# tomzzy1/ldbc_graphalytics_platforms_graphblas

Hardware: AMD Instinct MI355X
Metric: edges/sec (GTEPS) per algorithm at 1/2/4/8 GPUs; % HBM roofline (higher is better)
Workload: dtype f64; 1 GPU; PageRank SYN-8_5 (R-MAT scale 23, ef 40, seed 85, undirected); algorithm=pagerank, graph=SYN-8_5, n=8388608, nnz=628313590, parallelism=row1, partition=one rank, driver=device, hipGraph, exchange=device copies, roofline_events=timed steps, device=AMD Radeon Graphics (gfx950:sramecc+:xnack-), cus=256

## Files before the change

### ldbc_graphalytics_platforms_graphblas_amd/csrc/gx_pr.h

```cpp
#pragma once

#include <chrono>
#include <cstdio>
#include <cstdlib>
#include <vector>

#include <algorithm>

#include "gx_device.h"

namespace gx {

struct PlanClock {
    bool on = false, sync = true;
    hipStream_t s = nullptr;
    const char *what = "";
    std::chrono::steady_clock::time_point t;
    PlanClock(const char *w, hipStream_t st) : s(st), what(w) {
        const char *e = std::getenv("GX_PLAN_TIMES");
        on = e && std::atoi(e) != 0;
        sync = !(e && std::atoi(e) == 2);
        if (on) {
            if (sync) (void)hipStreamSynchronize(s);
            t = std::chrono::steady_clock::now();
        }
    }
    void mark(const char *phase) {
        if (!on) return;
        if (sync) (void)hipStreamSynchronize(s);
        const auto now = std::chrono::steady_clock::now();
        std::fprintf(stderr, "[plan %s] %-28s %8.2f ms\n", what, phase,
                     std::chrono::duration<double, std::milli>(now - t).count());
        t = now;
    }
};

struct RowBlock {
    int64_t nz_begin;
    int64_t nz_end;
    int32_t row_begin;
    int32_t row_end;
    int32_t split;
    int32_t seg;
};

struct SortedUnit {
    int64_t lo;
    int64_t hi;
    int64_t step;
    int64_t slab;
    int64_t nbeg;
    int32_t nsg;
    int32_t blk;
    int32_t part;
    int32_t unit;
    int32_t nunits;
    int32_t seg;
    int64_t z0, z1;
    int32_t r0, r1;
    int64_t pbeg;
    int32_t psg;
    int32_t pad;
};

struct CombStripe {
    int64_t slab;
    int32_t r0, nrows, s0, s1, k, dslot;
};

__device__ __forceinline__ void store_x(double *x_out, double *xd, int64_t live, int64_t row, double v) {
    if (row < live) x_out[row] = v;
    else xd[row - live] = v;
}

constexpr int kPullBlock = 256;
constexpr int kStreamNnz = 2048;
constexpr int kStreamRows = 256;
constexpr int kSegNnz = 8192;

struct PrPart {
    gx_ctx *ctx = nullptr;
    uint64_t n_global = 0;
    int nranks = 1, rank = 0;
    uint64_t rows = 0;
    uint64_t chunk = 0;
    uint64_t live = ~0ull;
    DBuf<double> xd;
    double damping = 0.85;
    DBuf<int64_t> rp_own;
    DBuf<int32_t> ci_own;
    const int64_t *rp = nullptr;
    const int32_t *ci = nullptr;
    DBuf<int32_t> outdeg_own;
    const int32_t *outdeg = nullptr;
    DBuf<RowBlock> blocks;
    uint32_t nblocks = 0;
    uint32_t nlong_blocks = 0;
    DBuf<int32_t> long_first;
    DBuf<int32_t> long_nseg;
    DBuf<double> long_part;
    DBuf<uint32_t> long_ticket;
    uint32_t nlong = 0, nsegs = 0;
    DBuf<int32_t> dlist;
    uint64_t nd = 0;
    bool d_range = false;
    int64_t d0 = 0;
    uint32_t dgrid = 0;
    DBuf<double> dpart;
    DBuf<uint32_t> dticket;
    DBuf<int32_t> sci;
    DBuf<uint32_t> spk;
    DBuf<uint32_t> gbase;
    DBuf<uint16_t> npk;
    DBuf<uint32_t> nbase;
    uint64_t nnarrow = 0;
    uint64_t ncodes = 0;
    uint32_t null_sg = 0;
    DBuf<uint32_t> ppk;
    DBuf<uint32_t> pbase;
    uint64_t npair = 0;
    uint64_t npfill = 0;
    uint64_t npslots = 0;
    uint32_t pnull_sg = 0;
    int sorted_nnz = 65536;
    int sorted_rows = 4096;
    int64_t unit_nnz = 0;
    DBuf<SortedUnit> units;
    uint32_t nunits = 0;
    DBuf<double> uslab;
    DBuf<uint32_t> uticket;
    bool comb_kernel = false;
    bool force_huge = false;
    DBuf<CombStripe> cstripes;
    uint32_t ncstripes = 0;
    DBuf<uint64_t> utimes;
    int utimes_launch = 0;
    int long_nnz = 65536;
    int sorted_lds = 0;
    int cache_policy = 0;
    uint32_t nt_col = 65536;
    uint32_t nsorted = 0, nlong_pad = 0;
    bool rows_desc = false;
    int queue_on = -1;
    DBuf<uint32_t> queue;
    bool fused_dangling = false;
    DBuf<int32_t> dslot;
    DBuf<double> fdpart;
    DBuf<uint32_t> fdticket;
    uint32_t ndblocks = 0;
    uint32_t iso_units = 0, iso_dblocks = 0;
    uint64_t iso_rows = 0;
    int kernel = 2;
    const int64_t *src_rp = nullptr;
    const int32_t *src_ci = nullptr;
    const int32_t *src_order = nullptr;
    const int32_t *src_perm = nullptr;
    UploadJob *job = nullptr;
    DBuf<int32_t> order;
    DBuf<double> xa, xb, rank_out, result;
    DBuf<int32_t> perm;
};

struct LengthRuns {
    std::vector<int64_t> pos, val, base;
    uint64_t n = 0;
    int64_t total = 0;
    size_t run(uint64_t i) const {
        return (size_t)(std::upper_bound(pos.begin(), pos.end(), (int64_t)i) - pos.begin()) - 1;
    }
    int64_t prefix(uint64_t i) const {
        if (i >= n) return total;
        const size_t k = run(i);
        return base[k] + ((int64_t)i - pos[k]) * val[k];
    }
    int64_t length(uint64_t i) const { return val[run(i)]; }
};

template <typename T>
struct HostView {
    const T *p = nullptr;
    size_t n = 0;
    const LengthRuns *runs = nullptr;
    bool prefix = false;
    template <typename Alloc>
    HostView(const std::vector<T, Alloc> &v) : p(v.data()), n(v.size()) {}
    HostView(const T *ptr, size_t count) : p(ptr), n(count) {}
    HostView(const LengthRuns *r, bool pre) : n(pre ? r->n + 1 : r->n), runs(r), prefix(pre) {}
    size_t size() const { return n; }
    T operator[](size_t i) const { return p ? p[i] : (T)(prefix ? runs->prefix(i) : runs->length(i)); }
};

int pr_plan(PrPart *p, HostView<int64_t> h_rp, const int64_t *d_rp,
            const int32_t *d_ci, const int32_t *d_outdeg, HostView<int32_t> h_outdeg);

int pr_plan_sorted(PrPart *p, HostView<int64_t> h_rp, HostView<int32_t> h_outdeg);
int pr_step_sorted(PrPart *p, const double *x_full, double *x_local, double *rank_out, hipStream_t s);
int pr_dangling(PrPart *p, double *x_local, hipStream_t s);

int pr_init(PrPart *p, double *x_local, hipStream_t s);
int pr_single_plan(gx_graph *g, PrPart **out);
constexpr int kPlanBlockRows = 16320;
constexpr int64_t kPlanBlockNnz = 32 << 20;

struct MultiBlocks {
    std::vector<std::vector<int32_t>> pos;
    std::vector<int32_t> slot;
    uint64_t chunk = 0;
    std::vector<int32_t> order, perm;
};
int pr_multi_blocks(const gx_csr *A, int directed, int ndev, MultiBlocks *out);
int pr_multi_interleave(const gx_csr *A, int ndev, MultiBlocks *out);

int pr_multi_plan(gx_graph *g, int ndev, int d, uint64_t chunk, double damping, const MultiBlocks *mb,
                  PrPart **out);
int pr_part_build(gx_ctx *ctx, uint64_t n_global, int nranks, int rank, uint64_t chunk, uint64_t live,
                  const std::vector<int64_t> &h_rp, const std::vector<int32_t> &ci, const std::vector<int32_t> &h_outdeg,
                  double damping, PrPart **out, bool force_huge = false);
int pr_part_build_rows(gx_ctx *ctx, const gx_csr *A, int nranks, int rank, uint64_t chunk,
                       const std::vector<int32_t> &rows, const int32_t *colmap, double damping, bool force_huge,
                       PrPart **out);
int pr_step(PrPart *p, const double *x_full, double *x_local, double *rank_out, hipStream_t s);

}
```

### ldbc_graphalytics_platforms_graphblas_amd/csrc/gx_pr_sorted.hip

```cpp
#include <algorithm>
#include <functional>
#include <queue>
#include <thread>
#include <type_traits>
#include <cstdio>
#include <cstdlib>
#include <cstring>

#include "gx_pr.h"
#include "gx_pr_bank.h"

namespace gx {
namespace {

constexpr int kRowBits = 14;
constexpr int kBS = 1024;
constexpr int kCombRows = (1 << kRowBits) / kBS;
constexpr int kU = 8;
constexpr int kRound = kBS * kU;
constexpr int kNSg = 512;
constexpr int kPSg = 256;
constexpr int kJunkRow = (1 << kRowBits) - kWave;
constexpr int kMaxBlockRows = kJunkRow;
static_assert(kMaxBlockRows == kPlanBlockRows, "gx_pr.h block rows");

struct SortedArgs {
    const RowBlock *blocks;
    const int32_t *ci;
    const int32_t *sci;
    const uint32_t *spk;
    const uint32_t *gbase;
    const int32_t *outdeg;
    const double *x_in;
    double *x_out;
    double *rank_out;
    int64_t chunk;
    int nranks;
    int zero_slot;
    int32_t zero_col;
    double teleport0, damping_over_n, damping;
    const int32_t *long_first;
    const int32_t *long_nseg;
    double *long_part;
    uint32_t *long_ticket;
    uint32_t nlong, nlong_pad;
    const int32_t *dslot;
    double *dpart;
    uint32_t *dticket;
    uint32_t ndblocks;
    double iso_rows;
    const SortedUnit *units;
    uint32_t nunits;
    double *uslab;
    uint32_t *uticket;
    uint64_t *utimes;
    const uint16_t *npk;
    const uint32_t *nbase;
    uint32_t null_sg;
    uint32_t nt_col;
    const uint32_t *ppk;
    const uint32_t *pbase;
    uint32_t pnull_sg;
    double *xd;
    int64_t live;
    uint32_t *queue;
    int comb;
    const CombStripe *cstripes;
};

__device__ __forceinline__ double sorted_epilogue(const SortedArgs &a, int64_t row, double s, double teleport) {
    const double r = teleport + s;
    if (a.rank_out) a.rank_out[row] = r;
    const int32_t deg = a.outdeg[row];
    store_x(a.x_out, a.xd, a.live, row, deg > 0 ? r / ((double)deg / a.damping) : r);
    return deg > 0 ? 0.0 : r;
}

__device__ __forceinline__ double epilogue_rows(const SortedArgs &a, int64_t r0, int nrows, const double *acc,
                                                double teleport) {
    constexpr int kB = 8;
    double d = 0.0;
    for (int i0 = threadIdx.x; i0 < nrows; i0 += kB * kBS) {
        int32_t deg[kB];
#pragma unroll
        for (int q = 0; q < kB; q++) {
            const int i = i0 + q * kBS;
            deg[q] = i < nrows ? a.outdeg[r0 + i] : 1;
        }
#pragma unroll
        for (int q = 0; q < kB; q++) {
            const int i = i0 + q * kBS;
            if (i >= nrows) break;
            const double r = teleport + (acc ? acc[i] : 0.0);
            if (a.rank_out) a.rank_out[r0 + i] = r;
            store_x(a.x_out, a.xd, a.live, r0 + i, deg[q] > 0 ? r / ((double)deg[q] / a.damping) : r);
            if (deg[q] == 0) d += r;
        }
    }
    return d;
}

template <int BS = kBS>
__device__ __forceinline__ void dangling_publish(const SortedArgs &a, int32_t slot, double d, double *wred, int *last,
                                                 double teleport) {
    const int tid = threadIdx.x;
    d = wave_sum(d);
    __syncthreads();
    if ((tid & (kWave - 1)) == 0) wred[tid / kWave] = d;
    __syncthreads();
    if (tid == 0) {
        double tot = 0.0;
#pragma unroll
        for (int w = 0; w < BS / kWave; w++) tot += wred[w];
        __hip_atomic_store(&a.dpart[slot], tot, __ATOMIC_RELAXED, __HIP_MEMORY_SCOPE_AGENT);
        __builtin_amdgcn_fence(__ATOMIC_RELEASE, "agent");
        asm volatile("s_waitcnt vmcnt(0)" ::: "memory");
        const uint32_t t = __hip_atomic_fetch_add(a.dticket, 1u, __ATOMIC_RELAXED, __HIP_MEMORY_SCOPE_AGENT);
        *last = t == a.ndblocks - 1;
    }
    __syncthreads();
    if (!*last) return;
    __builtin_amdgcn_fence(__ATOMIC_ACQUIRE, "agent");
    double v = 0.0;
    for (uint32_t j = tid; j < a.ndblocks; j += BS) v += __hip_atomic_load(&a.dpart[j], __ATOMIC_RELAXED, __HIP_MEMORY_SCOPE_AGENT);
    v = wave_sum(v);
    __syncthreads();
    if ((tid & (kWave - 1)) == 0) wred[tid / kWave] = v;
    __syncthreads();
    if (tid == 0) {
        double all = 0.0;
#pragma unroll
        for (int w = 0; w < BS / kWave; w++) all += wred[w];
        __hip_atomic_store(a.dticket, 0u, __ATOMIC_RELAXED, __HIP_MEMORY_SCOPE_AGENT);
        a.x_out[a.chunk - 1] = all + a.iso_rows * teleport;
    }
}

__device__ __forceinline__ void long_segment(const SortedArgs &a, const RowBlock &b, double *wred, double teleport) {
    const int tid = threadIdx.x;
    const int64_t zb = b.nz_begin, ze = b.nz_end;
    double s0 = 0.0, s1 = 0.0;
    for (int64_t k0 = zb + tid; k0 < ze; k0 += (int64_t)kU * kBS) {
        int32_t c[kU];
#pragma unroll
        for (int u = 0; u < kU; u++) c[u] = __builtin_nontemporal_load(a.ci + min(k0 + (int64_t)u * kBS, ze - 1));
        double g[kU];
#pragma unroll
        for (int u = 0; u < kU; u++) g[u] = a.x_in[c[u]];
#pragma unroll
        for (int u = 0; u < kU; u++)
            if (k0 + (int64_t)u * kBS < ze) ((u & 1) ? s1 : s0) += g[u];
    }
    const double s = wave_sum(s0 + s1);
    if ((tid & (kWave - 1)) == 0) wred[tid / kWave] = s;
    __syncthreads();
    if (tid != 0) return;
    double tot = 0.0;
#pragma unroll
    for (int w = 0; w < kBS / kWave; w++) tot += wred[w];
    const int32_t sp = b.split;
    const int32_t nseg = a.long_nseg[sp];
    if (nseg == 1) {
        sorted_epilogue(a, b.row_begin, tot, teleport);
        return;
    }
    const int32_t first = a.long_first[sp];
    __hip_atomic_store(&a.long_part[first + b.seg], tot, __ATOMIC_RELAXED, __HIP_MEMORY_SCOPE_AGENT);
    __builtin_amdgcn_fence(__ATOMIC_RELEASE, "agent");
    asm volatile("s_waitcnt vmcnt(0)" ::: "memory");
    const uint32_t t = __hip_atomic_fetch_add(&a.long_ticket[sp], 1u, __ATOMIC_RELAXED, __HIP_MEMORY_SCOPE_AGENT);
    if (t != (uint32_t)(nseg - 1)) return;
    __builtin_amdgcn_fence(__ATOMIC_ACQUIRE, "agent");
    double all = 0.0;
    for (int j = 0; j < nseg; j++)
        all += __hip_atomic_load(&a.long_part[first + j], __ATOMIC_RELAXED, __HIP_MEMORY_SCOPE_AGENT);
    __hip_atomic_store(&a.long_ticket[sp], 0u, __ATOMIC_RELAXED, __HIP_MEMORY_SCOPE_AGENT);
    sorted_epilogue(a, b.row_begin, all, teleport);
}

template <int CP>
__device__ __forceinline__ void gather_units(const SortedArgs &a, const RowBlock &b, int64_t lo64, int64_t hi64,
                                             double *acc, int64_t step64) {
    const int tid = threadIdx.x;
    const int64_t z0 = b.nz_begin;
    const int32_t lo = (int32_t)(lo64 - z0), hi = (int32_t)(hi64 - z0), step = (int32_t)step64;
    if (lo >= hi) return;
    const int32_t last = (int32_t)(b.nz_end - z0) - 1;
    const int32_t nsg = (last >> 8) + 1;
    const uint32_t span = (uint32_t)(hi - lo);
    const uint32_t *spk = a.spk + z0;
    const int32_t *sci = a.sci + z0;
    const uint32_t *sgb = a.gbase + b.seg;
    const int32_t zc = a.zero_col;
    const char *xb = reinterpret_cast<const char *>(a.x_in);
    const int lane = tid & (kWave - 1);
    constexpr int V = kU / 4;
    const int wave = tid >> 6;
    struct Rd {
        uint4 q[V];
        uint32_t bq;
    };
    struct Gt {
        double g[kU];
        uint32_t r[kU];
    };
    auto load = [&](Rd &d, int32_t R) {
        const int32_t sg0 = R + wave * V * 256;
#pragma unroll
        for (int v = 0; v < V; v++) {
            const int32_t sg = sg0 + v * 256;
            const gx_u32x4 *qa = reinterpret_cast<const gx_u32x4 *>(spk + min(sg + 4 * lane, last));
            const gx_u32x4 q4 = (CP & 1) ? __builtin_nontemporal_load(qa) : *qa;
            d.q[v] = make_uint4(q4.x, q4.y, q4.z, q4.w);
        }
        d.bq = sgb[min((sg0 >> 8) + (lane & (V - 1)), nsg - 1)];
    };
    auto issue = [&](const Rd &d, int32_t R, Gt &t) {
        int32_t c[kU];
        uint32_t sb[V], esc = 0;
#pragma unroll
        for (int v = 0; v < V; v++) {
            sb[v] = __builtin_amdgcn_readlane(d.bq, v);
            esc |= sb[v];
        }
#pragma unroll
        for (int v = 0; v < V; v++) {
            const uint32_t w4[4] = {d.q[v].x, d.q[v].y, d.q[v].z, d.q[v].w};
            const int32_t d0 = R + (wave * V + v) * 256 + 4 * lane - lo;
            const uint32_t base = sb[v] & 0x7fffffffu;
#pragma unroll
            for (int j = 0; j < 4; j++) {
                const int i = 4 * v + j;
                const bool ok = (uint32_t)(d0 + j) < span;
                t.r[i] = w4[j] & ((1u << kRowBits) - 1);
                asm volatile("" : "+v"(t.r[i]));
                c[i] = ok ? (int32_t)(base + (w4[j] >> kRowBits)) : zc;
            }
        }
        if (esc & 0x80000000u) {
#pragma unroll
            for (int v = 0; v < V; v++) {
                if (!(sb[v] & 0x80000000u)) continue;
#pragma unroll
                for (int j = 0; j < 4; j++) {
                    const int i = 4 * v + j;
                    const int32_t pos = R + (wave * V + v) * 256 + 4 * lane + j;
                    if ((uint32_t)(pos - lo) < span) c[i] = sci[pos];
                }
            }
            __builtin_amdgcn_s_waitcnt(0x0f70);
        }
#pragma unroll
        for (int i = 0; i < kU; i++) t.g[i] = *reinterpret_cast<const double *>(xb + ((uint32_t)c[i] << 3));
    };
    auto add = [&](const Gt &t) {
#pragma unroll
        for (int i = 0; i < kU; i++) atomicAdd(&acc[t.r[i]], t.g[i]);
    };
    const int32_t nr = (hi - lo + step - 1) / step;
    if (nr <= 0) return;
    Rd dA, dB;
    Gt tA, tB;
    int32_t R = lo;
    load(dA, R);
    load(dB, R + step);
    issue(dA, R, tA);
    __builtin_amdgcn_sched_barrier(0);
    load(dA, R + 2 * step);
    int32_t k = 1;
    for (; k + 1 < nr; k += 2) {
        __builtin_amdgcn_sched_barrier(0);
        issue(dB, R + step, tB);
        __builtin_amdgcn_sched_barrier(0);
        load(dB, R + 3 * step);
        __builtin_amdgcn_sched_barrier(0);
        add(tA);
        __builtin_amdgcn_sched_barrier(0);
        issue(dA, R + 2 * step, tA);
        __builtin_amdgcn_sched_barrier(0);
        load(dA, R + 4 * step);
        __builtin_amdgcn_sched_barrier(0);
        add(tB);
        R += 2 * step;
    }
    if (k < nr) {
        issue(dB, R + step, tB);
        add(tA);
        add(tB);
    } else {
        add(tA);
    }
}

__device__ __forceinline__ uint32_t wave_scan_incl(uint32_t v) {
    v += (uint32_t)__builtin_amdgcn_update_dpp(0, (int)v, 0x111, 0xf, 0xf, false);
    v += (uint32_t)__builtin_amdgcn_update_dpp(0, (int)v, 0x112, 0xf, 0xf, false);
    v += (uint32_t)__builtin_amdgcn_update_dpp(0, (int)v, 0x114, 0xf, 0xf, false);
    v += (uint32_t)__builtin_amdgcn_update_dpp(0, (int)v, 0x118, 0xf, 0xf, false);
    v += (uint32_t)__builtin_amdgcn_update_dpp(0, (int)v, 0x142, 0xa, 0xf, false);
    v += (uint32_t)__builtin_amdgcn_update_dpp(0, (int)v, 0x143, 0xc, 0xf, false);
    return v;
}

template <int CP>
__device__ __forceinline__ void gather_narrow(const SortedArgs &a, const SortedUnit &u, double *acc) {
    constexpr int W = kBS / kWave;
    const int32_t nrounds = (u.nsg + W - 1) / W;
    if (u.unit >= nrounds) return;
    const int32_t nr = (nrounds - u.unit + u.nunits - 1) / u.nunits;
    if (nr <= 0) return;
    const int tid = threadIdx.x;
    const int lane = tid & (kWave - 1);
    const int wave = tid >> 6;
    const uint32_t sg0 = (uint32_t)(u.nbeg / kNSg);
    const char *xb = reinterpret_cast<const char *>(a.x_in);
    typedef uint32_t u32x4 __attribute__((ext_vector_type(4)));
    struct Rd {
        u32x4 q;
        uint32_t base;
    };
    struct Gt {
        double g[kU];
        uint32_t r[kU];
    };
    auto load = [&](Rd &d, int32_t i) {
        const int32_t sg = (u.unit + i * u.nunits) * W + wave;
        const uint32_t g = sg < u.nsg ? sg0 + (uint32_t)sg : a.null_sg;
        const u32x4 *qa = reinterpret_cast<const u32x4 *>(a.npk + (size_t)g * kNSg) + lane;
        d.q = (CP & 1) ? __builtin_nontemporal_load(qa) : *qa;
        d.base = a.nbase[g];
    };
    auto issue = [&](const Rd &d, Gt &t) {
        const uint32_t w[4] = {d.q.x, d.q.y, d.q.z, d.q.w};
        uint32_t pk[2] = {0u, 0u};
#pragma unroll
        for (int k = 0; k < kU; k++) {
            const uint32_t c = (k & 1) ? (w[k >> 1] >> 16) : (w[k >> 1] & 0xffffu);
            pk[k >> 2] |= (c >> kRowBits) << (8 * (k & 3));
            t.r[k] = c & ((1u << kRowBits) - 1);
            asm volatile("" : "+v"(t.r[k]));
        }
        const uint32_t s0 = wave_scan_incl(pk[0]), s1 = wave_scan_incl(pk[1]);
        const uint32_t t0 = (uint32_t)__builtin_amdgcn_readlane((int)s0, kWave - 1);
        const uint32_t t1 = (uint32_t)__builtin_amdgcn_readlane((int)s1, kWave - 1);
        uint32_t bk = (uint32_t)__builtin_amdgcn_readfirstlane((int)d.base);
        const uint32_t b0 = bk;
        uint32_t col[kU];
#pragma unroll
        for (int k = 0; k < kU; k++) {
            const uint32_t sk = k < 4 ? s0 : s1, tk = k < 4 ? t0 : t1;
            col[k] = bk + ((sk >> (8 * (k & 3))) & 255u);
            bk += (tk >> (8 * (k & 3))) & 255u;
        }
        if ((CP & 4) && b0 >= a.nt_col) {
#pragma unroll
            for (int k = 0; k < kU; k++) t.g[k] = __builtin_nontemporal_load(reinterpret_cast<const double *>(xb + (col[k] << 3)));
        } else {
#pragma unroll
            for (int k = 0; k < kU; k++) t.g[k] = *reinterpret_cast<const double *>(xb + (col[k] << 3));
        }
    };
    auto add = [&](const Gt &t) {
#pragma unroll
        for (int k = 0; k < kU; k++) atomicAdd(&acc[t.r[k]], t.g[k]);
    };
    Rd dA, dB;
    Gt tA, tB;
    load(dA, 0);
    load(dB, 1);
    issue(dA, tA);
    __builtin_amdgcn_sched_barrier(0);
    load(dA, 2);
    int32_t k = 1;
    for (; k + 1 < nr; k += 2) {
        __builtin_amdgcn_sched_barrier(0);
        issue(dB, tB);
        __builtin_amdgcn_sched_barrier(0);
        load(dB, k + 2);
        __builtin_amdgcn_sched_barrier(0);
        add(tA);
        __builtin_amdgcn_sched_barrier(0);
        issue(dA, tA);
        __builtin_amdgcn_sched_barrier(0);
        load(dA, k + 3);
        __builtin_amdgcn_sched_barrier(0);
        add(tB);
    }
    if (k < nr) {
        issue(dB, tB);
        add(tA);
        add(tB);
    } else {
        add(tA);
    }
}

template <int CP>
__device__ __forceinline__ void gather_pairs(const SortedArgs &a, const SortedUnit &u, double *acc) {
    constexpr int W = kBS / kWave;
    constexpr int kS = kU / 2;
    const int32_t nrounds = (u.psg + W - 1) / W;
    if (u.unit >= nrounds) return;
    const int32_t nr = (nrounds - u.unit + u.nunits - 1) / u.nunits;
    const int tid = threadIdx.x;
    const int lane = tid & (kWave - 1);
    const int wave = tid >> 6;
    const uint32_t sg0 = (uint32_t)(u.pbeg / kPSg);
    const char *xb = reinterpret_cast<const char *>(a.x_in);
    typedef uint32_t u32x4 __attribute__((ext_vector_type(4)));
    typedef double d2 __attribute__((ext_vector_type(2)));
    struct Rd {
        u32x4 q;
        uint32_t base;
    };
    struct Gt {
        d2 g[kS];
        uint32_t r[kS];
    };
    auto load = [&](Rd &d, int32_t i) {
        const int32_t sg = (u.unit + i * u.nunits) * W + wave;
        const uint32_t g = sg < u.psg ? sg0 + (uint32_t)sg : a.pnull_sg;
        const u32x4 *qa = reinterpret_cast<const u32x4 *>(a.ppk + (size_t)g * kPSg) + lane;
        d.q = (CP & 1) ? __builtin_nontemporal_load(qa) : *qa;
        d.base = a.pbase[g];
    };
    auto issue = [&](const Rd &d, Gt &t) {
        const uint32_t w[kS] = {d.q.x, d.q.y, d.q.z, d.q.w};
        uint32_t pk = 0u;
#pragma unroll
        for (int k = 0; k < kS; k++) {
            pk |= (w[k] >> 30) << (8 * k);
            t.r[k] = w[k] & 0x3fffffffu;
            asm volatile("" : "+v"(t.r[k]));
        }
        const uint32_t sc = wave_scan_incl(pk);
        const uint32_t tot = (uint32_t)__builtin_amdgcn_readlane((int)sc, kWave - 1);
        uint32_t bk = (uint32_t)__builtin_amdgcn_readfirstlane((int)d.base);
        const uint32_t b0 = bk;
        uint32_t pr[kS];
#pragma unroll
        for (int k = 0; k < kS; k++) {
            pr[k] = bk + ((sc >> (8 * k)) & 255u);
            bk += (tot >> (8 * k)) & 255u;
        }
        if ((CP & 4) && 2u * b0 >= a.nt_col) {
#pragma unroll
            for (int k = 0; k < kS; k++) t.g[k] = __builtin_nontemporal_load(reinterpret_cast<const d2 *>(xb + (pr[k] << 4)));
        } else {
#pragma unroll
            for (int k = 0; k < kS; k++) t.g[k] = *reinterpret_cast<const d2 *>(xb + (pr[k] << 4));
        }
    };
    auto add = [&](const Gt &t) {
#pragma unroll
        for (int k = 0; k < kS; k++) {
            const uint32_t r = t.r[k];
            atomicAdd(&acc[(r >> 15) & ((1u << kRowBits) - 1)], (r & (1u << 29)) ? t.g[k].y : t.g[k].x);
            atomicAdd(&acc[r & ((1u << kRowBits) - 1)], (r & (1u << kRowBits)) ? t.g[k].y : t.g[k].x);
        }
    };
    Rd dA, dB;
    Gt tA, tB;
    load(dA, 0);
    load(dB, 1);
    issue(dA, tA);
    __builtin_amdgcn_sched_barrier(0);
    load(dA, 2);
    int32_t k = 1;
    for (; k + 1 < nr; k += 2) {
        __builtin_amdgcn_sched_barrier(0);
        issue(dB, tB);
        __builtin_amdgcn_sched_barrier(0);
        load(dB, k + 2);
        __builtin_amdgcn_sched_barrier(0);
        add(tA);
        __builtin_amdgcn_sched_barrier(0);
        issue(dA, tA);
        __builtin_amdgcn_sched_barrier(0);
        load(dA, k + 3);
        __builtin_amdgcn_sched_barrier(0);
        add(tB);
    }
    if (k < nr) {
        issue(dB, tB);
        add(tA);
        add(tB);
    } else {
        add(tA);
    }
}

template <bool TIMES, int CP>
__device__ __forceinline__ void pull_item(const SortedArgs &a, const uint32_t w, double *acc, double *wred, int &last,
                                          const double teleport) {
    const int tid = threadIdx.x;
    __shared__ uint64_t ts[2];
    if (TIMES && tid == 0) ts[0] = __builtin_amdgcn_s_memrealtime();
    auto stamp = [&]() {
        if (TIMES && tid == 0) {
            a.utimes[4 * w + 0] = ts[0];
            a.utimes[4 * w + 1] = ts[1];
            a.utimes[4 * w + 2] = __builtin_amdgcn_s_memrealtime();
            a.utimes[4 * w + 3] = (uint64_t)__builtin_amdgcn_s_getreg((3 << 11) | 20);
        }
    };
    if (a.zero_slot && w == 0 && tid == 0) a.x_out[a.chunk - 1] = a.iso_rows * teleport;
    if (w < a.nlong_pad) {
        if (w < a.nlong) long_segment(a, a.blocks[w], wred, teleport);
        stamp();
        return;
    }
    const SortedUnit u = a.units[w - a.nlong_pad];
    const RowBlock b = {u.z0, u.z1, u.r0, u.r1, -1, u.seg};
    const int nrows = b.row_end - b.row_begin;
    const bool empty = b.nz_begin == b.nz_end;
    if (!empty) {
        for (int i = tid; i < nrows; i += kBS) acc[i] = 0.0;
        __syncthreads();
        gather_pairs<CP>(a, u, acc);
        gather_narrow<CP>(a, u, acc);
        gather_units<CP>(a, b, u.lo, u.hi, acc, u.step);
        __syncthreads();
    }
    if (TIMES && tid == 0) ts[1] = __builtin_amdgcn_s_memrealtime();
    if (u.nunits > 1 && a.comb) {
        double *mine = a.uslab + u.slab + (int64_t)u.unit * nrows;
        for (int i = tid; i < nrows; i += kBS) mine[i] = acc[i];
        stamp();
        return;
    }
    if (u.nunits > 1) {
        double *mine = a.uslab + u.slab + (int64_t)u.unit * nrows;
        for (int i = tid; i < nrows; i += kBS)
            __hip_atomic_store(&mine[i], acc[i], __ATOMIC_RELAXED, __HIP_MEMORY_SCOPE_AGENT);
        asm volatile("s_waitcnt vmcnt(0)" ::: "memory");
        __syncthreads();
        if (tid == 0) {
            const uint32_t t = __hip_atomic_fetch_add(&a.uticket[u.part], 1u, __ATOMIC_RELAXED, __HIP_MEMORY_SCOPE_AGENT);
            last = t == (uint32_t)(u.nunits - 1);
            if (last) {
                __builtin_amdgcn_fence(__ATOMIC_ACQUIRE, "agent");
                asm volatile("s_waitcnt vmcnt(0)" ::: "memory");
                __hip_atomic_store(&a.uticket[u.part], 0u, __ATOMIC_RELAXED, __HIP_MEMORY_SCOPE_AGENT);
            }
        }
        __syncthreads();
        if (!last) {
            stamp();
            return;
        }
        const double *slabs = a.uslab + u.slab;
        if (2 * nrows <= kBS) {
            int S = 2;
            while (4 * S * nrows <= 2 * kBS && S < u.nunits) S *= 2;
            double *part = acc + (1 << (kRowBits - 1));
            const int r = tid % nrows, g = tid / nrows;
            if (g < S) {
                double s = 0.0;
                for (int j0 = g; j0 < u.nunits; j0 += kCombRows * S) {
                    double v[kCombRows];
#pragma unroll
                    for (int q = 0; q < kCombRows; q++) {
                        const int j = j0 + q * S;
                        v[q] = j < u.nunits ? slabs[(int64_t)j * nrows + r] : 0.0;
                    }
#pragma unroll
                    for (int q = 0; q < kCombRows; q++) s += v[q];
                }
                part[g * nrows + r] = s;
            }
            __syncthreads();
            if (tid < nrows) {
                double s = 0.0;
                for (int q = 0; q < S; q++) s += part[q * nrows + tid];
                acc[tid] = s;
            }
        } else
        for (int i0 = tid; i0 < nrows; i0 += kCombRows * kBS) {
            double s[kCombRows];
#pragma unroll
            for (int q = 0; q < kCombRows; q++) s[q] = 0.0;
            for (int j = 0; j < u.nunits; j++) {
                const double *sl = slabs + (int64_t)j * nrows;
                double v[kCombRows];
#pragma unroll
                for (int q = 0; q < kCombRows; q++) v[q] = i0 + q * kBS < nrows ? sl[i0 + q * kBS] : 0.0;
#pragma unroll
                for (int q = 0; q < kCombRows; q++) s[q] += v[q];
            }
#pragma unroll
            for (int q = 0; q < kCombRows; q++)
                if (i0 + q * kBS < nrows) acc[i0 + q * kBS] = s[q];
        }
    }
    double d = 0.0;
    if (empty)
        d = epilogue_rows(a, b.row_begin, nrows, nullptr, teleport);
    else
        d = epilogue_rows(a, b.row_begin, nrows, acc, teleport);
    if (a.dslot) {
        const int32_t slot = a.dslot[u.blk];
        if (slot >= 0) dangling_publish(a, slot, d, wred, &last, teleport);
    }
    stamp();
}

constexpr int kCombBS = 256;
__global__ __launch_bounds__(kCombBS) void k_pr_combine(SortedArgs a) {
    __shared__ double part[kCombBS];
    __shared__ double wred[kCombBS / kWave];
    __shared__ int last;
    double dsum = 0.0;
    for (int k = 0; k < a.nranks; k++) dsum += a.x_in[(int64_t)k * a.chunk + a.chunk - 1];
    const double teleport = a.teleport0 + a.damping_over_n * dsum;
    const CombStripe c = a.cstripes[blockIdx.x];
    const int rows = c.s1 - c.s0;
    int S = 1;
    while (2 * S * rows <= kCombBS && S < c.k) S *= 2;
    const int tid = threadIdx.x, r = tid % rows, g = tid / rows;
    double s = 0.0;
    if (g < S) {
        const double *sl = a.uslab + c.slab + c.s0 + r;
        for (int j0 = g; j0 < c.k; j0 += 16 * S) {
            double v[16];
#pragma unroll
            for (int q = 0; q < 16; q++) {
                const int j = j0 + q * S;
                v[q] = j < c.k ? sl[(int64_t)j * c.nrows] : 0.0;
            }
#pragma unroll
            for (int q = 0; q < 16; q++) s += v[q];
        }
    }
    if (S > 1) {
        if (g < S) part[g * rows + r] = s;
        __syncthreads();
        if (tid < rows) {
            s = 0.0;
            for (int q = 0; q < S; q++) s += part[q * rows + tid];
        }
    }
    double d = 0.0;
    if (tid < rows) d = sorted_epilogue(a, (int64_t)c.r0 + c.s0 + tid, s, teleport);
    if (c.dslot >= 0) dangling_publish<kCombBS>(a, c.dslot, d, wred, &last, teleport);
}

__device__ __forceinline__ uint32_t queue_fetch(uint32_t *q, uint32_t *slot) {
    if (__builtin_amdgcn_readfirstlane(threadIdx.x) < (uint32_t)kWave) {
        const uint32_t v = __hip_atomic_fetch_add(q, (threadIdx.x & (kWave - 1)) == 0 ? 1u : 0u, __ATOMIC_RELAXED,
                                                  __HIP_MEMORY_SCOPE_AGENT);
        *slot = __builtin_amdgcn_readfirstlane(v);
    }
    __syncthreads();
    const uint32_t w = __builtin_amdgcn_readfirstlane(*slot);
    __syncthreads();
    return w;
}

template <bool TIMES, int CP = 0, bool QUEUE = false>
__global__ __launch_bounds__(kBS, TIMES ? 1 : 4) void k_pr_pull_units(SortedArgs a) {
    extern __shared__ double acc[];
    __shared__ double wred[kBS / kWave];
    __shared__ int last;
    double dsum = 0.0;
    for (int k = 0; k < a.nranks; k++) dsum += a.x_in[(int64_t)k * a.chunk + a.chunk - 1];
    const double teleport = a.teleport0 + a.damping_over_n * dsum;
    if constexpr (!QUEUE) {
        pull_item<TIMES, CP>(a, blockIdx.x, acc, wred, last, teleport);
    } else {
        __shared__ uint32_t item;
        const uint32_t total = a.nlong_pad + a.nunits;
        for (;;) {
            const uint32_t w = queue_fetch(a.queue, &item);
            if (w >= total) break;
            pull_item<TIMES, CP>(a, w, acc, wred, last, teleport);
        }
        if (threadIdx.x == 0 &&
            __hip_atomic_fetch_add(&a.queue[1], 1u, __ATOMIC_RELAXED, __HIP_MEMORY_SCOPE_AGENT) == gridDim.x - 1) {
            __hip_atomic_store(&a.queue[0], 0u, __ATOMIC_RELAXED, __HIP_MEMORY_SCOPE_AGENT);
            __hip_atomic_store(&a.queue[1], 0u, __ATOMIC_RELAXED, __HIP_MEMORY_SCOPE_AGENT);
        }
    }
}

using PullKernel = void (*)(SortedArgs);
template <bool QUEUE>
PullKernel pull_kernel(bool times, int cache_policy) {
    if (times) return k_pr_pull_units<true, 0, QUEUE>;
    if (cache_policy == 5) return k_pr_pull_units<false, 5, QUEUE>;
    if (cache_policy == 1) return k_pr_pull_units<false, 1, QUEUE>;
    return k_pr_pull_units<false, 0, QUEUE>;
}

struct KeySrc {
    const int64_t *rp;
    int64_t rows;
    const int64_t *srp;
    const int32_t *sci;
    const int32_t *order;
    const int32_t *perm;
    const int32_t *seg_row;
    int32_t nseg;
    int colbits;
    int32_t segmask;
};

__global__ __launch_bounds__(256) void k_row_seg(const int32_t *__restrict__ seg_row, int32_t nseg, int32_t *rowseg) {
    for (int32_t sg = blockIdx.x; sg < nseg; sg += gridDim.x)
        for (int32_t r = seg_row[sg] + threadIdx.x; r < seg_row[sg + 1]; r += 256) rowseg[r] = sg;
}

constexpr int kKeyU = 4;

template <typename K>
__global__ __launch_bounds__(256) void k_sorted_keys(KeySrc k, int64_t nnz, const int64_t *__restrict__ srow,
                                                     int64_t nslabs, const int32_t *__restrict__ rowseg,
                                                     K *__restrict__ keys, uint16_t *__restrict__ vals) {
    const int lane = threadIdx.x & (kWave - 1);
    const int64_t nw = (int64_t)gridDim.x * (256 / kWave);
    const int64_t nch = (nslabs + kKeyU - 1) / kKeyU;
    for (int64_t ch = ((int64_t)blockIdx.x * 256 + threadIdx.x) / kWave; ch < nch; ch += nw) {
        int32_t i[kKeyU], sg[kKeyU], c0[kKeyU];
        int64_t rpi[kKeyU], sp[kKeyU];
        const int64_t e0 = ch * kKeyU * kWave + lane;
#pragma unroll
        for (int u = 0; u < kKeyU; u++) {
            const int64_t sl = min(ch * kKeyU + u, nslabs - 1);
            i[u] = (int32_t)slab_row_of(k.rp, srow, k.rows, sl, min(e0 + u * kWave, nnz - 1), lane);
        }
#pragma unroll
        for (int u = 0; u < kKeyU; u++) {
            sg[u] = rowseg[i[u]];
            rpi[u] = k.rp[i[u]];
            sp[u] = k.srp[k.order ? k.order[i[u]] : i[u]];
        }
#pragma unroll
        for (int u = 0; u < kKeyU; u++) c0[u] = k.sci[sp[u] + (min(e0 + u * kWave, nnz - 1) - rpi[u])];
#pragma unroll
        for (int u = 0; u < kKeyU; u++) {
            const uint32_t c = (uint32_t)(k.perm ? k.perm[c0[u]] : c0[u]);
            const int64_t e = e0 + u * kWave;
            if (e < nnz) {
                keys[e] = ((K)(sg[u] & k.segmask) << k.colbits) | (K)c;
                vals[e] = (uint16_t)(i[u] - k.seg_row[sg[u]]);
            }
        }
    }
}

template <typename K>
__global__ __launch_bounds__(256) void k_scatter_keys(KeySrc k, int64_t n_src, const int64_t *__restrict__ ssrow,
                                                      int64_t sl0, int64_t sl1, int64_t nnz,
                                                      const int32_t *__restrict__ rowseg, K *__restrict__ keys,
                                                      uint16_t *__restrict__ vals) {
    const int lane = threadIdx.x & (kWave - 1);
    const int64_t nw = (int64_t)gridDim.x * (256 / kWave);
    const int64_t nslabs_src = (nnz + kWave - 1) / kWave;
    for (int64_t sl = sl0 + ((int64_t)blockIdx.x * 256 + threadIdx.x) / kWave; sl < sl1; sl += nw) {
        const int64_t e = sl * kWave + lane;
        const int64_t ee = min(e, nnz - 1);
        const int64_t u = slab_row_of(k.srp, ssrow, n_src, min(sl, nslabs_src - 1), ee, lane);
        const int32_t i = k.perm[u];
        const int32_t sg = rowseg[i];
        const int64_t dst = k.rp[i] + (ee - k.srp[u]);
        const uint32_t c = (uint32_t)k.perm[k.sci[ee]];
        if (e < nnz) {
            keys[dst] = ((K)(sg & k.segmask) << k.colbits) | (K)c;
            vals[dst] = (uint16_t)(i - k.seg_row[sg]);
        }
    }
}

struct SegDesc {
    int64_t z0, z1;
    int32_t gseg;
    int32_t pad;
};

constexpr int64_t kPackChunk = 4096;
struct PackChunk {
    int64_t z0;
    int32_t seg;
    int32_t pad;
};

template <typename K>
__global__ __launch_bounds__(256) void k_sorted_pack(const SegDesc *__restrict__ segs, const PackChunk *__restrict__ chunks,
                                                     int64_t nchunks, const K *__restrict__ keys,
                                                     const uint16_t *__restrict__ vals, uint32_t colmask,
                                                     int32_t *__restrict__ sci, uint32_t *__restrict__ spk,
                                                     uint32_t *__restrict__ gbase) {
    for (int64_t c = blockIdx.x; c < nchunks; c += gridDim.x) {
        const PackChunk pc = chunks[c];
        const SegDesc sg = segs[pc.seg];
        const int64_t z1 = min(pc.z0 + kPackChunk, sg.z1);
#pragma unroll 4
        for (int64_t g0 = pc.z0; g0 < z1; g0 += 256) {
            const int64_t e = g0 + threadIdx.x;
            const bool in = e < z1;
            const uint32_t col = in ? (uint32_t)keys[e] & colmask : 0u;
            if (in) sci[e] = (int32_t)col;
            if (sg.gseg < 0 || !in) continue;
            const int64_t q = (g0 - sg.z0) >> 8;
            const uint32_t base = (uint32_t)keys[g0] & colmask;
            const uint32_t lastc = (uint32_t)keys[min(g0 + 255, sg.z1 - 1)] & colmask;
            const bool esc = lastc - base >= (1u << (32 - kRowBits));
            const uint32_t row = vals[e];
            spk[e] = esc ? row : ((col - base) << kRowBits) | row;
            if (threadIdx.x == 0) gbase[sg.gseg + q] = esc ? (base | 0x80000000u) : base;
        }
    }
}

__global__ __launch_bounds__(256) void k_sorted_laneperm(const RowBlock *__restrict__ blocks, const uint32_t *__restrict__ nsplit,
                                                         uint32_t *spk, int32_t *sci) {
    const RowBlock b = blocks[blockIdx.y];
    const int64_t z0 = b.nz_begin + 256 * (int64_t)nsplit[blockIdx.y], ngroups = (b.nz_end - z0) >> 6;
    const int lane = threadIdx.x & (kWave - 1);
    const int64_t wave = ((int64_t)blockIdx.x * blockDim.x + threadIdx.x) / kWave;
    const int64_t waves = (int64_t)gridDim.x * blockDim.x / kWave;
    for (int64_t g = wave; g < ngroups; g += waves) {
        const int64_t e = z0 + (g << 6) + lane;
        const uint32_t p = spk[e];
        const int32_t c = sci[e];
        const uint32_t row = p & ((1u << kRowBits) - 1);
        const uint32_t key = ((row & 15u) << 1) | ((row >> 4) & 1u);
        uint32_t rank = 0;
        for (uint32_t k = 0; k < 32; k++) {
            const uint64_t m = __ballot(key == k);
            if (k < key) rank += (uint32_t)__popcll(m);
            else if (k == key) rank += (uint32_t)__popcll(m & ((1ull << lane) - 1ull));
        }
        const int64_t dst = z0 + (g << 6) + 4 * (rank >> 2) + (rank & 3);
        spk[dst] = p;
        sci[dst] = c;
    }
}

constexpr int kBankTile = 2048, kBankBS = 256, kBankPer = kBankTile / kBankBS;
__global__ __launch_bounds__(kBankBS) void k_bank_order(const RowBlock *__restrict__ blocks, const uint32_t *__restrict__ qsplit,
                                                        const uint32_t *__restrict__ nsplit, uint32_t *spk, int32_t *sci) {
    __shared__ uint32_t cnt2[kBankTile / 2][kBankClasses / 2];
    __shared__ int32_t wred[2][kBankBS / kWave];
    const RowBlock b = blocks[blockIdx.y];
    const int64_t z0 = b.nz_begin, N = b.nz_end - z0;
    const int64_t Nq = min(N, (int64_t)qsplit[blockIdx.y] << 8), Np = min(N, (int64_t)nsplit[blockIdx.y] << 8);
    const int64_t ntiles = (Np + kBankTile - 1) / kBankTile;
    const int tid = threadIdx.x, lane = tid & (kWave - 1), wave = tid / kWave;
    for (int64_t g = blockIdx.x; g < ntiles; g += gridDim.x) {
        const int64_t t0 = g * kBankTile;
        const int32_t nin = (int32_t)min<int64_t>(kBankTile, Np - t0);
        uint32_t p[kBankPer], key[kBankPer];
        int32_t c[kBankPer], s0[kBankPer], s1[kBankPer];
        bool head[kBankPer];
        for (int w = tid; w < kBankTile / 2 * (kBankClasses / 2); w += kBankBS) (&cnt2[0][0])[w] = 0u;
        const int32_t i0 = tid * kBankPer;
        uint32_t prevkey = 0;
        if (i0 > 0 && i0 < nin) {
            const int64_t e = t0 + i0 - 1;
            prevkey = e < Nq ? (uint32_t)sci[z0 + e] >> 1 : (uint32_t)sci[z0 + e];
        }
#pragma unroll
        for (int j = 0; j < kBankPer; j++) {
            const int32_t i = i0 + j;
            const bool in = i < nin;
            p[j] = in ? spk[z0 + t0 + i] : 0u;
            c[j] = in ? sci[z0 + t0 + i] : 0;
            key[j] = t0 + i < Nq ? (uint32_t)c[j] >> 1 : (uint32_t)c[j];
        }
        int32_t last = -1;
#pragma unroll
        for (int j = 0; j < kBankPer; j++) {
            const int32_t i = i0 + j;
            head[j] = i == 0 || i >= nin || t0 + i == Nq || key[j] != (j ? key[j - 1] : prevkey);
            if (head[j]) last = i;
            s0[j] = last;
        }
        int32_t first = kBankTile;
#pragma unroll
        for (int j = kBankPer - 1; j >= 0; j--) {
            s1[j] = first;
            if (head[j]) first = i0 + j;
        }
        int32_t m0 = last, m1 = first;
#pragma unroll
        for (int d = 1; d < kWave; d <<= 1) {
            const int32_t v0 = __shfl_up(m0, d, kWave), v1 = __shfl_down(m1, d, kWave);
            if (lane >= d) m0 = max(m0, v0);
            if (lane + d < kWave) m1 = min(m1, v1);
        }
        if (lane == kWave - 1) wred[0][wave] = m0;
        if (lane == 0) wred[1][wave] = m1;
        int32_t before = __shfl_up(m0, 1, kWave), after = __shfl_down(m1, 1, kWave);
        if (lane == 0) before = -1;
        if (lane == kWave - 1) after = kBankTile;
        __syncthreads();
        for (int w = 0; w < kBankBS / kWave; w++) {
            if (w < wave) before = max(before, wred[0][w]);
            if (w > wave) after = min(after, wred[1][w]);
        }
        uint32_t rank[kBankPer];
#pragma unroll
        for (int j = 0; j < kBankPer; j++) {
            if (s0[j] < 0) s0[j] = before;
            s1[j] = min(s1[j], after);
            rank[j] = 0;
            if (s1[j] - s0[j] > 1) {
                const uint32_t cls = p[j] & (uint32_t)(kBankClasses - 1);
                const uint32_t old = atomicAdd(&cnt2[s0[j] >> 1][cls >> 1], 1u << (16 * (cls & 1)));
                rank[j] = (old >> (16 * (cls & 1))) & 0xffffu;
            }
        }
        __syncthreads();
#pragma unroll
        for (int j = 0; j < kBankPer; j++) {
            const uint32_t n = (uint32_t)(s1[j] - s0[j]);
            if (n <= 1) continue;
            uint32_t cnt[kBankClasses];
#pragma unroll
            for (int k = 0; k < kBankClasses / 2; k++) {
                const uint32_t w = cnt2[s0[j] >> 1][k];
                cnt[2 * k] = w & 0xffffu;
                cnt[2 * k + 1] = w >> 16;
            }
            const uint32_t k = bank_deal_pos(cnt, p[j] & (uint32_t)(kBankClasses - 1), rank[j]);
            const bool pairs = t0 + s0[j] < Nq;
            const int64_t dst = z0 + t0 + s0[j] + (pairs ? bank_pair_pos(k, n) : k);
            spk[dst] = p[j];
            if (pairs) sci[dst] = c[j];
        }
        __syncthreads();
    }
}


__device__ __forceinline__ uint32_t narrow_fillers(const int32_t *sci, int64_t z0, int64_t e, uint32_t *step) {
    const uint32_t c = (uint32_t)sci[e];
    const uint32_t s0 = e > z0 ? c - (uint32_t)sci[e - 1] : 0u;
    *step = s0;
    return s0 > 3 ? (s0 + 2) / 3 - 1 : 0u;
}

__device__ __forceinline__ uint32_t wave_total(uint32_t v) {
    return (uint32_t)__builtin_amdgcn_readlane((int)wave_scan_incl(v), kWave - 1);
}

__global__ __launch_bounds__(256) void k_narrow_cost(const RowBlock *__restrict__ blocks, const int32_t *__restrict__ sci,
                                                     const uint32_t *__restrict__ qsplit, uint32_t *__restrict__ fill) {
    const RowBlock b = blocks[blockIdx.y];
    const int64_t z0 = b.nz_begin, N = b.nz_end - z0, ng = (N + 255) >> 8;
    const int64_t Q = qsplit[blockIdx.y], zq = z0 + (Q << 8);
    const int lane = threadIdx.x & (kWave - 1);
    const int64_t waves = (int64_t)gridDim.x * blockDim.x / kWave;
    for (int64_t g = Q + ((int64_t)blockIdx.x * blockDim.x + threadIdx.x) / kWave; g < ng; g += waves) {
        uint32_t d = 0, st;
#pragma unroll
        for (int j = 0; j < 4; j++) {
            const int64_t e = (g << 8) + 4 * lane + j;
            if (e < N) d += narrow_fillers(sci, zq, z0 + e, &st);
        }
        d = wave_total(d);
        if (lane == 0) fill[b.seg + g] = d;
    }
}

__global__ __launch_bounds__(1024) void k_narrow_split(const RowBlock *__restrict__ blocks, const uint32_t *__restrict__ fill,
                                                       const uint32_t *__restrict__ codes, int w4,
                                                       const uint32_t *__restrict__ qsplit,
                                                       int enable, int64_t min_entries, uint32_t *__restrict__ nsplit,
                                                       uint32_t *__restrict__ ncode,
                                                       uint32_t *__restrict__ noff) {
    __shared__ int64_t sben[1024], scod[1024];
    __shared__ int64_t bestv[1024];
    __shared__ int32_t besti[1024];
    const RowBlock b = blocks[blockIdx.x];
    const int64_t N = b.nz_end - b.nz_begin, ng = (N + 255) >> 8;
    const int t = threadIdx.x;
    const int64_t per = (ng + 1023) / 1024, g0 = min(ng, t * per), g1 = min(ng, g0 + per);
    const int64_t Q = qsplit ? (int64_t)qsplit[blockIdx.x] : 0;
    auto cnt = [&](int64_t g) { return min<int64_t>(256, N - (g << 8)); };
    auto benefit = [&](int64_t g) { return g < Q ? 0 : 4 * cnt(g) - (int64_t)w4 * (int64_t)fill[b.seg + g]; };
    auto ncodes = [&](int64_t g) {
        return g < Q ? 0 : codes ? (int64_t)codes[b.seg + g] : cnt(g) + (int64_t)fill[b.seg + g];
    };
    int64_t ben = 0, cod = 0;
    for (int64_t g = g0; g < g1; g++) {
        ben += benefit(g);
        cod += ncodes(g);
    }
    sben[t] = ben;
    scod[t] = cod;
    __syncthreads();
    for (int o = 1; o < 1024; o <<= 1) {
        const int64_t a1 = t >= o ? sben[t - o] : 0, a2 = t >= o ? scod[t - o] : 0;
        __syncthreads();
        sben[t] += a1;
        scod[t] += a2;
        __syncthreads();
    }
    int64_t pb = sben[t] - ben, pc = scod[t] - cod;
    int64_t bv = 0;
    int32_t bi = (int32_t)Q;
    for (int64_t g = g0; g < g1; g++) {
        noff[b.seg + g] = (uint32_t)pc;
        pb += benefit(g);
        pc += ncodes(g);
        if (pb > bv) {
            bv = pb;
            bi = (int32_t)(g + 1);
        }
    }
    bestv[t] = bv;
    besti[t] = bi;
    __syncthreads();
    for (int o = 512; o > 0; o >>= 1) {
        if (t < o) {
            const int64_t v2 = bestv[t + o];
            const int32_t i2 = besti[t + o];
            if (v2 > bestv[t] || (v2 == bestv[t] && i2 < besti[t])) {
                bestv[t] = v2;
                besti[t] = i2;
            }
        }
        __syncthreads();
    }
    if (t == 0) {
        const int32_t P = (enable && N >= min_entries) ? besti[0] : (int32_t)Q;
        nsplit[blockIdx.x] = (uint32_t)P;
        ncode[blockIdx.x] = P == Q ? 0u : (uint32_t)(P < ng ? noff[b.seg + P] : (uint32_t)scod[1023]);
    }
}

__global__ void k_narrow_fill(uint16_t *__restrict__ npk, uint64_t ncodes, uint32_t *__restrict__ nbase, uint32_t null_sg,
                              uint32_t zero_col) {
    for (uint64_t p = (uint64_t)blockIdx.x * blockDim.x + threadIdx.x; p < ncodes; p += (uint64_t)gridDim.x * blockDim.x)
        npk[p] = (uint16_t)(kJunkRow + ((p >> 3) & (kWave - 1)));
    if (blockIdx.x == 0 && threadIdx.x == 0) nbase[null_sg] = zero_col;
}

__global__ __launch_bounds__(256) void k_narrow_emit(const RowBlock *__restrict__ blocks, const int32_t *__restrict__ sci,
                                                     const uint32_t *__restrict__ spk, const uint32_t *__restrict__ qsplit,
                                                     const uint32_t *__restrict__ nsplit,
                                                     const uint32_t *__restrict__ ncode, const uint32_t *__restrict__ noff,
                                                     const int64_t *__restrict__ nbeg, uint16_t *__restrict__ npk,
                                                     uint32_t *__restrict__ nbase) {
    const RowBlock b = blocks[blockIdx.y];
    const int64_t z0 = b.nz_begin, N = b.nz_end - z0, P = nsplit[blockIdx.y];
    const int64_t Q = qsplit[blockIdx.y], zq = z0 + (Q << 8);
    const int64_t nb = nbeg[blockIdx.y], C = ncode[blockIdx.y];
    const int lane = threadIdx.x & (kWave - 1);
    const int64_t waves = (int64_t)gridDim.x * blockDim.x / kWave;
    if (P > Q && blockIdx.x == 0 && threadIdx.x == 0) nbase[nb / kNSg] = (uint32_t)sci[zq];
    for (int64_t g = Q + ((int64_t)blockIdx.x * blockDim.x + threadIdx.x) / kWave; g < P; g += waves) {
        uint32_t fl[4], st[4], n = 0;
#pragma unroll
        for (int j = 0; j < 4; j++) {
            const int64_t e = (g << 8) + 4 * lane + j;
            fl[j] = e < N ? narrow_fillers(sci, zq, z0 + e, &st[j]) : 0u;
            n += e < N ? fl[j] + 1 : 0u;
        }
        int64_t pos = nb + noff[b.seg + g] + (wave_scan_incl(n) - n);
        auto put = [&](uint32_t step, uint32_t row, uint32_t col_after) {
            npk[(pos & ~(int64_t)(kNSg - 1)) + (pos & (kWave - 1)) * 8 + ((pos >> 6) & 7)] = (uint16_t)((step << kRowBits) | row);
            const int64_t rel = pos - nb + 1;
            if ((rel & (kNSg - 1)) == 0 && rel < C) nbase[(pos + 1) / kNSg] = col_after;
            pos++;
        };
#pragma unroll
        for (int j = 0; j < 4; j++) {
            const int64_t e = (g << 8) + 4 * lane + j;
            if (e >= N) continue;
            const uint32_t c = (uint32_t)sci[z0 + e];
            uint32_t at = c - st[j];
            for (uint32_t f = 0; f < fl[j]; f++) {
                at += 3;
                put(3u, (uint32_t)(kJunkRow + (pos & (kWave - 1))), at);
            }
            put(c - at, spk[z0 + e] & ((1u << kRowBits) - 1), c);
        }
    }
}


struct PairLane {
    uint32_t pair[4], col[4], next[4];
    uint32_t step[4], sf[4];
    bool in[4], start[4], lead[4], half[4];
};

__device__ __forceinline__ void pair_lane(const int32_t *__restrict__ sci, int64_t z0, int64_t N, int64_t Nq, int64_t g,
                                          int lane, PairLane &o) {
    const int64_t i0 = (g << 8) + 4 * lane;
    uint32_t c[6];
#pragma unroll
    for (int j = 0; j < 6; j++) c[j] = (uint32_t)sci[z0 + min(max(i0 + j - 1, (int64_t)0), N - 1)];
    const int64_t f = g << 8;
    const uint32_t pf = (uint32_t)sci[z0 + f] >> 1;
    int64_t gs = f;
    if (f > 0 && ((uint32_t)sci[z0 + f - 1] >> 1) == pf) {
        int64_t lo = 0, hi = f;
        while (lo < hi) {
            const int64_t mid = (lo + hi) >> 1;
            if (((uint32_t)sci[z0 + mid] >> 1) >= pf) hi = mid;
            else lo = mid + 1;
        }
        gs = lo;
    }
    int32_t ls = -1;
#pragma unroll
    for (int j = 0; j < 4; j++) {
        const int64_t i = i0 + j;
        o.in[j] = i < Nq;
        o.col[j] = c[j + 1];
        o.next[j] = c[j + 2];
        o.pair[j] = c[j + 1] >> 1;
        o.start[j] = o.in[j] && (i == 0 || (c[j] >> 1) != o.pair[j]);
        if (o.start[j]) ls = 4 * lane + j;
    }
    int32_t m = ls;
#pragma unroll
    for (int d = 1; d < kWave; d <<= 1) {
        const int32_t v = __shfl_up(m, d, kWave);
        if (lane >= d) m = max(m, v);
    }
    int32_t before = __shfl_up(m, 1, kWave);
    if (lane == 0) before = -1;
    int64_t rs = before >= 0 ? f + before : gs;
#pragma unroll
    for (int j = 0; j < 4; j++) {
        const int64_t i = i0 + j;
        if (o.start[j]) rs = i;
        o.lead[j] = o.in[j] && (((i - rs) & 1) == 0);
        o.half[j] = o.lead[j] && (i + 1 >= Nq || (o.next[j] >> 1) != o.pair[j]);
        const uint32_t s0 = (o.start[j] && i > 0) ? o.pair[j] - (c[j] >> 1) : 0u;
        o.sf[j] = s0 > 3 ? (s0 + 2) / 3 - 1 : 0u;
        o.step[j] = s0 - 3 * o.sf[j];
    }
}

__global__ __launch_bounds__(256) void k_pair_cost(const RowBlock *__restrict__ blocks, const int32_t *__restrict__ sci,
                                                   uint32_t *__restrict__ slots, uint32_t *__restrict__ fill) {
    const RowBlock b = blocks[blockIdx.y];
    const int64_t z0 = b.nz_begin, N = b.nz_end - z0, ng = (N + 255) >> 8;
    const int lane = threadIdx.x & (kWave - 1);
    const int64_t waves = (int64_t)gridDim.x * blockDim.x / kWave;
    for (int64_t g = ((int64_t)blockIdx.x * blockDim.x + threadIdx.x) / kWave; g < ng; g += waves) {
        PairLane pl;
        pair_lane(sci, z0, N, N, g, lane, pl);
        uint32_t ns = 0, nf = 0;
#pragma unroll
        for (int j = 0; j < 4; j++) {
            ns += (pl.lead[j] ? 1u : 0u) + (pl.start[j] ? pl.sf[j] : 0u);
            nf += (pl.half[j] ? 1u : 0u) + (pl.start[j] ? 2 * pl.sf[j] : 0u);
        }
        ns = wave_total(ns);
        nf = wave_total(nf);
        if (lane == 0) {
            slots[b.seg + g] = ns;
            fill[b.seg + g] = nf;
        }
    }
}

__global__ void k_pair_fill(uint32_t *__restrict__ ppk, uint64_t nslots, uint32_t *__restrict__ pbase, uint32_t null_sg,
                            uint32_t zero_pair) {
    for (uint64_t p = (uint64_t)blockIdx.x * blockDim.x + threadIdx.x; p < nslots; p += (uint64_t)gridDim.x * blockDim.x) {
        const uint32_t junk = (uint32_t)(kJunkRow + ((p >> 2) & (kWave - 1)));
        ppk[p] = (junk << 15) | junk;
    }
    if (blockIdx.x == 0 && threadIdx.x == 0) pbase[null_sg] = zero_pair;
}

__global__ __launch_bounds__(256) void k_pair_emit(const RowBlock *__restrict__ blocks, const int32_t *__restrict__ sci,
                                                   const uint32_t *__restrict__ spk, const uint32_t *__restrict__ qsplit,
                                                   const uint32_t *__restrict__ pcount, const uint32_t *__restrict__ poff,
                                                   const int64_t *__restrict__ pbeg, uint32_t *__restrict__ ppk,
                                                   uint32_t *__restrict__ pbase, unsigned long long *__restrict__ nfill) {
    const RowBlock b = blocks[blockIdx.y];
    const int64_t z0 = b.nz_begin, N = b.nz_end - z0, Q = qsplit[blockIdx.y];
    const int64_t Nq = min(N, Q << 8);
    const int64_t pb = pbeg[blockIdx.y], C = pcount[blockIdx.y];
    const int lane = threadIdx.x & (kWave - 1);
    const int64_t waves = (int64_t)gridDim.x * blockDim.x / kWave;
    constexpr uint32_t kRowMask = (1u << kRowBits) - 1;
    if (Q > 0 && blockIdx.x == 0 && threadIdx.x == 0) pbase[pb / kPSg] = (uint32_t)sci[z0] >> 1;
    for (int64_t g = ((int64_t)blockIdx.x * blockDim.x + threadIdx.x) / kWave; g < Q; g += waves) {
        PairLane pl;
        pair_lane(sci, z0, N, Nq, g, lane, pl);
        uint32_t n = 0, nf = 0;
#pragma unroll
        for (int j = 0; j < 4; j++) {
            n += (pl.lead[j] ? 1u : 0u) + (pl.start[j] ? pl.sf[j] : 0u);
            nf += (pl.half[j] ? 1u : 0u) + (pl.start[j] ? 2 * pl.sf[j] : 0u);
        }
        int64_t pos = pb + poff[b.seg + g] + (wave_scan_incl(n) - n);
        nf = wave_total(nf);
        if (lane == 0 && nf) atomicAdd(nfill, (unsigned long long)nf);
        auto put = [&](uint32_t step, uint32_t ha, uint32_t hb, uint32_t pair_after) {
            ppk[(pos & ~(int64_t)(kPSg - 1)) + (pos & (kWave - 1)) * 4 + ((pos >> 6) & 3)] = (step << 30) | (ha << 15) | hb;
            const int64_t rel = pos - pb + 1;
            if ((rel & (kPSg - 1)) == 0 && rel < C) pbase[(pos + 1) / kPSg] = pair_after;
            pos++;
        };
#pragma unroll
        for (int j = 0; j < 4; j++) {
            if (!pl.lead[j]) continue;
            const int64_t e = (g << 8) + 4 * lane + j;
            uint32_t step = 0;
            if (pl.start[j]) {
                uint32_t at = pl.pair[j] - pl.step[j] - 3 * pl.sf[j];
                for (uint32_t f = 0; f < pl.sf[j]; f++) {
                    at += 3;
                    const uint32_t junk = (uint32_t)(kJunkRow + (pos & (kWave - 1)));
                    put(3u, junk, junk, at);
                }
                step = pl.step[j];
            }
            const uint32_t ha = ((pl.col[j] & 1u) << kRowBits) | (spk[z0 + e] & kRowMask);
            const uint32_t hb = pl.half[j] ? (uint32_t)(kJunkRow + (pos & (kWave - 1)))
                                           : ((pl.next[j] & 1u) << kRowBits) | (spk[z0 + e + 1] & kRowMask);
            put(step, ha, hb, pl.pair[j]);
        }
    }
}

int env_int(const char *name, int dflt, int lo, int hi) {
    if (const char *e = std::getenv(name)) {
        const int v = std::atoi(e);
        if (v >= lo && v <= hi) return v;
    }
    return dflt;
}

struct UnitCost {
    double rate = 2900.0, row = 0.002, fixed = 1.5, slab = 0.0005;
    int model = 0;
    double rt = 2.0;
};

double pr_unit_makespan(const std::vector<int64_t> &ents, const std::vector<int64_t> &effs, const std::vector<int64_t> &rws,
                        const std::vector<int64_t> &lsegs, int64_t t, int cus, bool by_cost, const UnitCost &uc) {
    const double kRate = uc.rate, kRow = uc.row, kFixed = uc.fixed, kSlab = uc.slab;
    std::vector<double> cost;
    for (size_t i = 0; i < ents.size(); i++) {
        const int64_t E = ents[i];
        const int64_t k = std::max<int64_t>(1, std::min((E + kRound - 1) / kRound, ((by_cost ? effs[i] : E) + t - 1) / t));
        if (uc.model == 1) {
            const double c = (double)effs[i] / (double)k / kRate + kRow * (double)rws[i] + kFixed +
                             (k > 1 ? kSlab * (double)rws[i] : 0.0);
            for (int64_t j = 0; j + 1 < k; j++) cost.push_back(c);
            cost.push_back(c + (k > 1 ? uc.rt * std::ceil((double)k * (double)rws[i] / (double)(1 << kRowBits)) : 0.0));
            continue;
        }
        const double c = (double)effs[i] / (double)k / kRate + kRow * (double)rws[i] + kFixed +
                         (k > 1 ? kSlab * (double)rws[i] * (double)k : 0.0);
        for (int64_t j = 0; j < k; j++) cost.push_back(c);
    }
    for (int64_t e : lsegs) cost.push_back((double)e / kRate + kFixed);
    std::sort(cost.begin(), cost.end(), std::greater<double>());
    std::priority_queue<double, std::vector<double>, std::greater<double>> slots;
    for (int i = 0; i < std::max(1, cus); i++) slots.push(0.0);
    double span = 0.0;
    for (double c : cost) {
        const double f = slots.top() + c;
        slots.pop();
        slots.push(f);
        span = std::max(span, f);
    }
    return span;
}

}

int pr_plan_sorted(PrPart *p, HostView<int64_t> h_rp, HostView<int32_t> h_outdeg) {
    const int64_t rows = (int64_t)h_rp.size() - 1;
    const uint64_t nnz = (uint64_t)h_rp[rows];
    const int64_t cus = std::max(1, p->ctx->num_cus);
    const double per_cu = std::max(1.0, (double)nnz / (double)cus);
    const bool huge = per_cu > (double)(2 << 20) || env_int("GX_PR_HUGE", 0, 0, 1) == 1 || p->force_huge;
    const bool piece = huge && p->nranks > 1;
    const int rmax = kMaxBlockRows;
    p->sorted_rows = env_int("GX_PR_SORTED_ROWS", huge ? rmax : 4096, 64, rmax);
    int64_t pow2 = 1 << 14;
    while (pow2 < (1 << 24) && (double)(2 * pow2) <= per_cu * 1.41421356) pow2 *= 2;
    const int64_t bdef = piece ? kPlanBlockNnz
                       : huge ? std::min<int64_t>(32 << 20, 16 * pow2)
                              : std::min<int64_t>(per_cu > 384.0 * 1024 ? 4 << 20 : 1 << 20, 4 * pow2);
    const int64_t B = env_int("GX_PR_BLOCK_NNZ", (int)bdef, 1024, 1 << 30);
    p->long_nnz = env_int("GX_PR_LONG_NNZ", (int)std::max<int64_t>(B / 4, kRound), 1024, 1 << 30);
    p->sorted_nnz = (int)B;
    const uint64_t xbytes = (uint64_t)p->chunk * (uint64_t)std::max(1, p->nranks) * sizeof(double);
    p->cache_policy = env_int("GX_PR_CP", xbytes >= (32ull << 20) ? 5 : 0, 0, 5);
    if (p->cache_policy != 0 && p->cache_policy != 1) p->cache_policy = 5;
    p->nt_col = (uint32_t)env_int("GX_PR_NT_COL", 65536, 0, 1 << 30);
    PlanClock clk("sorted", p->ctx->stream);
    const int64_t R = p->sorted_rows, LT = std::max<int64_t>(p->long_nnz, 1);
    std::vector<RowBlock> longb, sortb;
    std::vector<int32_t> lfirst, lnseg;
    std::vector<std::pair<int64_t, int32_t>> longrows;
    int32_t nsegs = 0;
    int64_t r = 0;
    if (p->rows_desc) {
        while (r < rows && h_rp[r + 1] - h_rp[r] > LT) {
            longrows.push_back({h_rp[r + 1] - h_rp[r], (int32_t)r});
            r++;
        }
        while (r < rows) {
            const int64_t start = r, lim = std::min<int64_t>(rows, start + R);
            const int64_t limit = h_rp[start] + B;
            int64_t lo = start + 1, hi = lim + 1;
            while (lo < hi) {
                const int64_t mid = (lo + hi) / 2;
                if (h_rp[mid] > limit) hi = mid;
                else lo = mid + 1;
            }
            r = std::max<int64_t>(start + 1, lo - 1);
            sortb.push_back({h_rp[start], h_rp[r], (int32_t)start, (int32_t)r, -1, 0});
        }
    }
    while (r < rows) {
        const int64_t len = h_rp[r + 1] - h_rp[r];
        if (len > LT) {
            longrows.push_back({len, (int32_t)r});
            r++;
            continue;
        }
        const int64_t start = r;
        int64_t nz = 0;
        while (r < rows && r - start < R) {
            const int64_t l = h_rp[r + 1] - h_rp[r];
            if (l > LT || nz + l > B) break;
            nz += l;
            r++;
        }
        sortb.push_back({h_rp[start], h_rp[r], (int32_t)start, (int32_t)r, -1, 0});
    }
    int64_t maxrows = 1;
    for (const RowBlock &b : sortb) maxrows = std::max<int64_t>(maxrows, b.row_end - b.row_begin);
    int64_t ngroups = 0;
    for (RowBlock &b : sortb) {
        b.seg = (int32_t)ngroups;
        ngroups += (b.nz_end - b.nz_begin + 255) / 256;
    }
    std::stable_sort(longrows.begin(), longrows.end(), [](const auto &x, const auto &y) { return x.first > y.first; });
    for (const auto &lr : longrows) {
        const int32_t row = lr.second;
        const int32_t nseg = (int32_t)((lr.first + kSegNnz - 1) / kSegNnz);
        const int32_t sp = (int32_t)lfirst.size();
        lfirst.push_back(nsegs);
        lnseg.push_back(nseg);
        for (int32_t s = 0; s < nseg; s++) {
            const int64_t zb = h_rp[row] + (int64_t)s * kSegNnz;
            longb.push_back({zb, std::min(zb + kSegNnz, h_rp[row + 1]), row, row + 1, sp, s});
        }
        nsegs += nseg;
    }
    p->sorted_lds = (int)(maxrows * sizeof(double));
    std::vector<RowBlock> all(longb);
    all.insert(all.end(), sortb.begin(), sortb.end());
    p->nblocks = (uint32_t)all.size();
    p->nlong_blocks = (uint32_t)longb.size();
    p->nlong = (uint32_t)lfirst.size();
    p->nsegs = (uint32_t)nsegs;
    GX_TRY(p->blocks.alloc(std::max<size_t>(all.size(), 1)));
    GX_TRY(p->long_first.alloc(std::max<size_t>(lfirst.size(), 1)));
    GX_TRY(p->long_nseg.alloc(std::max<size_t>(lnseg.size(), 1)));
    GX_TRY(p->long_part.alloc(std::max<size_t>(nsegs, 1)));
    GX_TRY(p->long_ticket.alloc(std::max<size_t>(lfirst.size(), 1)));
    if (!all.empty())
        GX_HIP_TRY(hipMemcpy(p->blocks.p, all.data(), all.size() * sizeof(RowBlock), hipMemcpyHostToDevice));
    if (!lfirst.empty()) {
        GX_HIP_TRY(hipMemcpy(p->long_first.p, lfirst.data(), lfirst.size() * 4, hipMemcpyHostToDevice));
        GX_HIP_TRY(hipMemcpy(p->long_nseg.p, lnseg.data(), lnseg.size() * 4, hipMemcpyHostToDevice));
    }
    GX_HIP_TRY(hipMemset(p->long_ticket.p, 0, p->long_ticket.n * 4));
    clk.mark("blocks (host)");

    GX_TRY(p->sci.alloc(std::max<uint64_t>(nnz, 1), 16));
    GX_TRY(p->spk.alloc(std::max<uint64_t>(nnz, 1), 16));
    GX_TRY(p->gbase.alloc(std::max<int64_t>(ngroups, 1), 16));
    hipStream_t s = p->ctx->stream;
    const RowBlock *d_sort = p->blocks.p + longb.size();
    std::vector<uint32_t> h_nsplit(sortb.size(), 0), h_ncode(sortb.size(), 0);
    std::vector<int64_t> h_nbeg(sortb.size(), 0);
    std::vector<uint32_t> h_psplit(sortb.size(), 0), h_pcount(sortb.size(), 0);
    std::vector<int64_t> h_pbeg(sortb.size(), 0);
    p->ncodes = 0;
    p->nnarrow = 0;
    p->npair = p->npfill = p->npslots = 0;
    const bool pairs_on = env_int("GX_PR_PAIRS", huge && !piece ? 1 : 0, 0, 1) == 1;
    if (pairs_on && (p->chunk & 1)) return fail(GX_INVALID_VALUE, "pr_plan_sorted: pair slots need an even chunk");
    DBuf<int32_t> d_seg_row;
    DBuf<SegDesc> d_segd;
    DBuf<int64_t> srow;
    DBuf<int32_t> d_rowseg;
    DBuf<PackChunk> d_pch;
    DBuf<uint32_t> d_fill, d_noff, d_nsplit, d_ncode;
    DBuf<int64_t> d_nbeg;
    DBuf<uint32_t> d_pslots, d_pfill, d_poff, d_psplit, d_pcount;
    DBuf<int64_t> d_pbeg;
    DBuf<unsigned long long> d_npfill;
    if (nnz > 0) {
        std::vector<std::pair<int32_t, int32_t>> order_;
        for (size_t i = 0; i < sortb.size(); i++) order_.push_back({sortb[i].row_begin, (int32_t)i});
        for (size_t j = 0; j < longrows.size(); j++) order_.push_back({longrows[j].second, -1 - (int32_t)j});
        std::sort(order_.begin(), order_.end());
        std::vector<int32_t> seg_row;
        std::vector<SegDesc> segd;
        for (const auto &o : order_) {
            const int32_t r0 = o.first;
            const bool blk = o.second >= 0;
            const int32_t r1 = blk ? sortb[o.second].row_end : r0 + 1;
            if (h_rp[r0] == h_rp[r1]) continue;
            seg_row.push_back(r0);
            segd.push_back({h_rp[r0], h_rp[r1], blk ? sortb[o.second].seg : -1, 0});
        }
        seg_row.push_back((int32_t)rows);
        int colbits = 1;
        const uint64_t ncols = p->nranks == 1 ? std::max<uint64_t>(p->n_global, 1) : p->chunk * (uint64_t)p->nranks;
        while ((1ull << colbits) < ncols) colbits++;
        int segbits = 1;
        while ((1ull << segbits) < segd.size()) segbits++;
        GX_TRY(d_seg_row.alloc(seg_row.size()));
        GX_TRY(d_segd.alloc(segd.size()));
        GX_HIP_TRY(hipMemcpyAsync(d_seg_row.p, seg_row.data(), seg_row.size() * 4, hipMemcpyHostToDevice, s));
        GX_HIP_TRY(hipMemcpyAsync(d_segd.p, segd.data(), segd.size() * sizeof(SegDesc), hipMemcpyHostToDevice, s));
        const bool narrow = colbits <= 31 && !env_int("GX_PR_WIDE_KEYS", 0, 0, 1);
        const int gbits = narrow ? std::min({segbits, 32 - colbits, env_int("GX_PR_SORT_GROUP_BITS", 32, 1, 32)}) : segbits;
        const KeySrc ks{p->rp, rows, p->src_rp, p->src_ci, p->src_order, p->src_perm, d_seg_row.p,
                        (int32_t)segd.size(), colbits, (int32_t)((1ll << gbits) - 1)};
        const int64_t nslabs = (int64_t)((nnz + kWave - 1) / kWave);
        GX_TRY(srow.alloc(nslabs + 1));
        GX_TRY(slab_rows(p->rp, rows, nslabs, srow.p, s));
        GX_TRY(d_rowseg.alloc(std::max<int64_t>(rows, 1)));
        hipLaunchKernelGGL(k_row_seg, dim3((unsigned)std::min<size_t>(segd.size(), 65535)), dim3(256), 0, s, d_seg_row.p,
                           (int32_t)segd.size(), d_rowseg.p);
        GX_TRY(check_launch("k_row_seg"));
        std::vector<PackChunk> pch;
        for (size_t g = 0; g < segd.size(); g++)
            for (int64_t z = segd[g].z0; z < segd[g].z1; z += kPackChunk) pch.push_back({z, (int32_t)g, 0});
        GX_TRY(d_pch.alloc(std::max<size_t>(pch.size(), 1)));
        if (!pch.empty())
            GX_HIP_TRY(hipMemcpyAsync(d_pch.p, pch.data(), pch.size() * sizeof(PackChunk), hipMemcpyHostToDevice, s));
        clk.mark("segments + slab rows");
        const unsigned kgrid = grid_for((uint64_t)((nslabs + kKeyU - 1) / kKeyU) * kWave, 256, 16384);
        const unsigned pgrid = (unsigned)std::min<size_t>(std::max<size_t>(pch.size(), 1), 1u << 20);
        const uint32_t colmask = (uint32_t)((1ull << colbits) - 1);
        const size_t kb = narrow ? 4 : 8, align = 256;
        auto up = [&](size_t x) { return (x + align - 1) / align * align; };
        const size_t kbytes = up((size_t)nnz * kb), vbytes = up((size_t)nnz * 2);
        char *scr = nullptr;
        GX_TRY(plan_scratch(2 * kbytes + 2 * vbytes, reinterpret_cast<void **>(&scr)));
        uint16_t *v0 = reinterpret_cast<uint16_t *>(scr + 2 * kbytes), *v1 = reinterpret_cast<uint16_t *>(scr + 2 * kbytes + vbytes);
        clk.mark("key buffers");
        auto key_pass = [&](auto *kk) -> int {
            using K = std::remove_pointer_t<decltype(kk)>;
            if (!p->job) {
                hipLaunchKernelGGL(k_sorted_keys<K>, dim3(kgrid), dim3(256), 0, s, ks, (int64_t)nnz, srow.p, nslabs,
                                   d_rowseg.p, kk, v0);
                return check_launch("k_sorted_keys");
            }
            const int64_t n_src = (int64_t)p->n_global;
            DBuf<int64_t> ssrow;
            GX_TRY(ssrow.alloc(nslabs + 1));
            GX_TRY(slab_rows(p->src_rp, n_src, nslabs, ssrow.p, s));
            UploadJob *job = p->job;
            for (size_t c = 0; c < job->ev.size(); c++) {
                GX_TRY(job->wait_chunk((int)c));
                GX_HIP_TRY(hipStreamWaitEvent(s, job->ev[c], 0));
                const int64_t e0 = c ? job->end[c - 1] : 0, e1 = job->end[c];
                const int64_t sl0 = e0 / kWave, sl1 = (e1 + kWave - 1) / kWave;
                hipLaunchKernelGGL(k_scatter_keys<K>, dim3(grid_for((uint64_t)(sl1 - sl0) * kWave, 256, 4096)), dim3(256),
                                   0, s, ks, n_src, ssrow.p, sl0, sl1, (int64_t)nnz, d_rowseg.p, kk, v0);
                GX_TRY(check_launch("k_scatter_keys"));
            }
            GX_TRY(job->join());
            GX_HIP_TRY(hipStreamSynchronize(s));
            return GX_SUCCESS;
        };
        if (narrow) {
            uint32_t *k0 = reinterpret_cast<uint32_t *>(scr), *k1 = reinterpret_cast<uint32_t *>(scr + kbytes);
            GX_TRY(key_pass(k0));
            clk.mark("keys");
            const size_t G = (size_t)1 << gbits;
            for (size_t g0 = 0; g0 < segd.size(); g0 += G) {
                const size_t g1 = std::min(segd.size(), g0 + G) - 1;
                const int64_t z0 = segd[g0].z0, z1 = segd[g1].z1;
                GX_TRY(sort_pairs_u32_u16(k0 + z0, k1 + z0, v0 + z0, v1 + z0, (size_t)(z1 - z0), gbits + colbits, s));
            }
            clk.mark("sort");
            hipLaunchKernelGGL(k_sorted_pack<uint32_t>, dim3(pgrid), dim3(256), 0, s, d_segd.p, d_pch.p,
                               (int64_t)pch.size(), k1, v1, colmask, p->sci.p, p->spk.p, p->gbase.p);
        } else {
            uint64_t *k0 = reinterpret_cast<uint64_t *>(scr), *k1 = reinterpret_cast<uint64_t *>(scr + kbytes);
            GX_TRY(key_pass(k0));
            GX_TRY(sort_pairs_u64_u16(k0, k1, v0, v1, (size_t)nnz, segbits + colbits, s));
            hipLaunchKernelGGL(k_sorted_pack<uint64_t>, dim3(pgrid), dim3(256), 0, s, d_segd.p, d_pch.p,
                               (int64_t)pch.size(), k1, v1, colmask, p->sci.p, p->spk.p, p->gbase.p);
        }
        GX_TRY(check_launch("k_sorted_pack"));
        clk.mark("keys + sort + pack");
        if (!sortb.empty()) {
            const unsigned nsb = (unsigned)sortb.size();
            GX_TRY(d_fill.alloc(std::max<int64_t>(ngroups, 1)));
            GX_TRY(d_noff.alloc(std::max<int64_t>(ngroups, 1)));
            GX_TRY(d_nsplit.alloc(nsb));
            GX_TRY(d_ncode.alloc(nsb));
            GX_TRY(d_nbeg.alloc(nsb));
            GX_TRY(d_psplit.alloc(nsb));
            GX_TRY(d_pcount.alloc(nsb));
            GX_TRY(d_pbeg.alloc(nsb));
            GX_TRY(d_npfill.alloc(1));
            GX_HIP_TRY(hipMemsetAsync(d_psplit.p, 0, nsb * 4, s));
            GX_HIP_TRY(hipMemsetAsync(d_npfill.p, 0, sizeof(unsigned long long), s));
            if (pairs_on) {
                GX_TRY(d_pslots.alloc(std::max<int64_t>(ngroups, 1)));
                GX_TRY(d_pfill.alloc(std::max<int64_t>(ngroups, 1)));
                GX_TRY(d_poff.alloc(std::max<int64_t>(ngroups, 1)));
                hipLaunchKernelGGL(k_pair_cost, dim3(64, nsb), dim3(256), 0, s, d_sort, p->sci.p, d_pslots.p, d_pfill.p);
                GX_TRY(check_launch("k_pair_cost"));
                hipLaunchKernelGGL(k_narrow_split, dim3(nsb), dim3(1024), 0, s, d_sort, d_pfill.p, d_pslots.p,
                                   env_int("GX_PR_PAIR_FILL_COST", 48, 0, 1 << 20), (const uint32_t *)nullptr, 1,
                                   (int64_t)env_int("GX_PR_PAIR_MIN", 0, 0, 1 << 30), d_psplit.p, d_pcount.p, d_poff.p);
                GX_TRY(check_launch("k_narrow_split (pairs)"));
                GX_HIP_TRY(hipMemcpyAsync(h_psplit.data(), d_psplit.p, nsb * 4, hipMemcpyDeviceToHost, s));
                GX_HIP_TRY(hipMemcpyAsync(h_pcount.data(), d_pcount.p, nsb * 4, hipMemcpyDeviceToHost, s));
            }
            hipLaunchKernelGGL(k_narrow_cost, dim3(64, nsb), dim3(256), 0, s, d_sort, p->sci.p, d_psplit.p, d_fill.p);
            GX_TRY(check_launch("k_narrow_cost"));
            hipLaunchKernelGGL(k_narrow_split, dim3(nsb), dim3(1024), 0, s, d_sort, d_fill.p, (const uint32_t *)nullptr, 4,
                               d_psplit.p, env_int("GX_PR_NARROW", 1, 0, 1),
                               (int64_t)env_int("GX_PR_NARROW_MIN", 0, 0, 1 << 30), d_nsplit.p, d_ncode.p, d_noff.p);
            GX_TRY(check_launch("k_narrow_split"));
            GX_HIP_TRY(hipMemcpyAsync(h_nsplit.data(), d_nsplit.p, nsb * 4, hipMemcpyDeviceToHost, s));
            GX_HIP_TRY(hipMemcpyAsync(h_ncode.data(), d_ncode.p, nsb * 4, hipMemcpyDeviceToHost, s));
            GX_HIP_TRY(hipStreamSynchronize(s));
            uint64_t run = 0, prun = 0;
            for (size_t i = 0; i < sortb.size(); i++) {
                const int64_t E = sortb[i].nz_end - sortb[i].nz_begin;
                const int64_t Ep = std::min<int64_t>((int64_t)h_psplit[i] * 256, E);
                h_nbeg[i] = (int64_t)run;
                run += ((uint64_t)h_ncode[i] + kNSg - 1) / kNSg * kNSg;
                p->nnarrow += (uint64_t)(std::min<int64_t>((int64_t)h_nsplit[i] * 256, E) - Ep);
                h_pbeg[i] = (int64_t)prun;
                prun += ((uint64_t)h_pcount[i] + kPSg - 1) / kPSg * kPSg;
                p->npair += (uint64_t)Ep;
            }
            if (env_int("GX_PR_BANK_ORDER", huge && !piece ? 1 : 0, 0, 1) == 1) {
                clk.mark("prefix splits");
                hipLaunchKernelGGL(k_bank_order, dim3(64, nsb), dim3(kBankBS), 0, s, d_sort, d_psplit.p, d_nsplit.p, p->spk.p,
                                   p->sci.p);
                GX_TRY(check_launch("k_bank_order"));
                clk.mark("bank order");
            }
            p->pnull_sg = (uint32_t)(prun / kPSg);
            p->npslots = prun + kPSg;
            GX_TRY(p->ppk.alloc(p->npslots, 16));
            GX_TRY(p->pbase.alloc(p->npslots / kPSg));
            hipLaunchKernelGGL(k_pair_fill, dim3(grid_for(p->npslots, 256, 16384)), dim3(256), 0, s, p->ppk.p, p->npslots,
                               p->pbase.p, p->pnull_sg, (uint32_t)((p->chunk - 2) >> 1));
            GX_TRY(check_launch("k_pair_fill"));
            if (p->npair) {
                GX_HIP_TRY(hipMemcpyAsync(d_pbeg.p, h_pbeg.data(), nsb * 8, hipMemcpyHostToDevice, s));
                hipLaunchKernelGGL(k_pair_emit, dim3(64, nsb), dim3(256), 0, s, d_sort, p->sci.p, p->spk.p, d_psplit.p,
                                   d_pcount.p, d_poff.p, d_pbeg.p, p->ppk.p, p->pbase.p, d_npfill.p);
                GX_TRY(check_launch("k_pair_emit"));
                unsigned long long nf = 0;
                GX_HIP_TRY(hipMemcpyAsync(&nf, d_npfill.p, sizeof nf, hipMemcpyDeviceToHost, s));
                GX_HIP_TRY(hipStreamSynchronize(s));
                p->npfill = nf;
            }
            p->null_sg = (uint32_t)(run / kNSg);
            p->ncodes = run + kNSg;
            GX_TRY(p->npk.alloc(p->ncodes, 16));
            GX_TRY(p->nbase.alloc(p->ncodes / kNSg));
            GX_HIP_TRY(hipMemcpyAsync(d_nbeg.p, h_nbeg.data(), nsb * 8, hipMemcpyHostToDevice, s));
            hipLaunchKernelGGL(k_narrow_fill, dim3(grid_for(p->ncodes, 256, 16384)), dim3(256), 0, s, p->npk.p, p->ncodes,
                               p->nbase.p, p->null_sg, (uint32_t)(p->chunk - 2));
            GX_TRY(check_launch("k_narrow_fill"));
            hipLaunchKernelGGL(k_narrow_emit, dim3(64, nsb), dim3(256), 0, s, d_sort, p->sci.p, p->spk.p, d_psplit.p, d_nsplit.p,
                               d_ncode.p, d_noff.p, d_nbeg.p, p->npk.p, p->nbase.p);
            GX_TRY(check_launch("k_narrow_emit"));
            clk.mark("narrow codes");
        }
        if (env_int("GX_PR_LANEPERM", 1, 0, 1) && !sortb.empty()) {
            hipLaunchKernelGGL(k_sorted_laneperm, dim3(64, (unsigned)sortb.size()), dim3(256), 0, s, d_sort, d_nsplit.p,
                               p->spk.p, p->sci.p);
            GX_TRY(check_launch("k_sorted_laneperm"));
        }
    }
    p->ci = p->sci.p;
    clk.mark("laneperm");
    p->nsorted = (uint32_t)sortb.size();
    p->nlong_pad = (p->nlong_blocks + 7u) & ~7u;
    int64_t T = 0;
    p->nunits = 0;
    const int64_t wide_cost4 = env_int("GX_PR_WIDE_COST", piece ? 11 : huge ? 24 : 4, 4, 64);
    const bool cost_codes = env_int("GX_PR_COST_CODES", piece ? 1 : 0, 0, 1) == 1;
    const int64_t fill_cost4 = env_int("GX_PR_FILL_COST", 4, 0, 64);
    const int64_t pair_cost4 = env_int("GX_PR_PAIR_COST", 4, 1, 64);
    auto eff_entries = [&](int64_t i) -> int64_t {
        const int64_t E = sortb[i].nz_end - sortb[i].nz_begin;
        const int64_t Ep = std::min<int64_t>(E, 256 * (int64_t)h_psplit[i]);
        const int64_t Enp = std::min<int64_t>(E, 256 * (int64_t)h_nsplit[i]);
        const int64_t En = Enp - Ep;
        const int64_t fill = cost_codes ? std::max<int64_t>(0, (int64_t)h_ncode[i] - En) : 0;
        const int64_t pent = cost_codes ? std::max<int64_t>(Ep, 2 * (int64_t)h_pcount[i]) : Ep;
        return pent * pair_cost4 / 4 + En + fill * fill_cost4 / 4 + (E - Enp) * wide_cost4 / 4;
    };
    const bool unit_by_cost = env_int("GX_PR_UNIT_BY_COST", huge ? 1 : 0, 0, 1) == 1;
    p->comb_kernel = env_int("GX_PR_COMBINE", piece ? 1 : 0, 0, 1) == 1;
    bool long_dangling = false;
    for (const RowBlock &b : longb) long_dangling |= h_outdeg[b.row_begin] == 0;
    const bool iso_on = env_int("GX_PR_ISO_CLOSED", 1, 0, 1) == 1 && p->nd > 0 && !long_dangling;
    auto iso_block = [&](const RowBlock &b) {
        if (!iso_on || b.nz_begin != b.nz_end || b.row_end <= b.row_begin) return false;
        if ((uint64_t)b.row_begin >= p->live) return true;
        return p->d_range && b.row_begin >= p->d0 && b.row_end <= p->d0 + (int64_t)p->nd;
    };
    p->iso_units = p->iso_dblocks = 0;
    p->iso_rows = 0;
    std::vector<CombStripe> stripes;
    std::vector<char> multi(longb.size() + sortb.size(), 0);
    if (sortb.empty()) GX_HIP_TRY(hipStreamSynchronize(s));
    if (!sortb.empty()) {
        if (std::getenv("GX_PR_UNIT_NNZ")) {
            T = env_int("GX_PR_UNIT_NNZ", 65536, 1024, 1 << 30);
        } else if (!huge && !env_int("GX_PR_UNIT_SIM", 0, 0, 1)) {
            T = std::max<int64_t>(kRound, (B / 4 + kRound - 1) / kRound * kRound);
        } else {
            std::vector<int64_t> ents, effs, rws, lsegs;
            for (const RowBlock &b : sortb) {
                ents.push_back(b.nz_end - b.nz_begin);
                effs.push_back(eff_entries(&b - sortb.data()));
                rws.push_back(b.row_end - b.row_begin);
            }
            for (const RowBlock &b : longb) lsegs.push_back(b.nz_end - b.nz_begin);
            double best = 0.0;
            const int64_t emax = *std::max_element(ents.begin(), ents.end());
            std::vector<int64_t> cand;
            for (int64_t t = kRound; t <= std::max<int64_t>(kRound, emax);
                 t = t < 64 * kRound ? t + kRound : (t + t / 25 + kRound - 1) / kRound * kRound)
                cand.push_back(t);
            std::vector<double> span(cand.size());
            UnitCost uc;
            if (piece) {
                uc.rate = 5650.0;
                uc.row = 0.0;
                uc.fixed = 8.3;
                uc.slab = 0.0002;
                uc.model = 1;
                uc.rt = p->comb_kernel ? 0.0 : 2.0;
            }
            uc.rate = (double)env_int("GX_PR_SIM_RATE", (int)uc.rate, 100, 1 << 20);
            uc.row = 1e-6 * (double)env_int("GX_PR_SIM_ROW_PS", (int)(uc.row * 1e6), 0, 1 << 20);
            uc.slab = 1e-6 * (double)env_int("GX_PR_SIM_SLAB_PS", (int)(uc.slab * 1e6), 0, 1 << 20);
            uc.model = env_int("GX_PR_SIM_MODEL", uc.model, 0, 1);
            uc.rt = 1e-3 * (double)env_int("GX_PR_SIM_RT_NS", (int)(uc.rt * 1e3), 0, 1 << 20);
            uc.fixed = 1e-3 * (double)env_int("GX_PR_SIM_FIXED_NS", (int)(uc.fixed * 1e3), 0, 1 << 20);
            const int nth = (int)std::max<size_t>(1, std::min<size_t>({8, cand.size(),
                                                                       (size_t)std::max(1u, std::thread::hardware_concurrency())}));
            std::vector<std::thread> th;
            for (int w = 0; w < nth; w++)
                th.emplace_back([&, w]() {
                    for (size_t i = (size_t)w; i < cand.size(); i += (size_t)nth)
                        span[i] = pr_unit_makespan(ents, effs, rws, lsegs, cand[i], (int)cus, unit_by_cost, uc);
                });
            for (auto &x : th) x.join();
            for (size_t i = 0; i < cand.size(); i++)
                if (T == 0 || span[i] < best * 0.999) {
                    best = span[i];
                    T = cand[i];
                }
            if (env_int("GX_PR_VERBOSE", 0, 0, 3))
                std::fprintf(stderr, "[gx_pr] unit size %lld: simulated launch %.1f us\n", (long long)T, best);
            if (env_int("GX_PR_VERBOSE", 0, 0, 3) >= 2) {
                std::vector<std::pair<double, size_t>> top;
                for (size_t i = 0; i < ents.size(); i++) {
                    const int64_t k = std::max<int64_t>(1, std::min((ents[i] + kRound - 1) / kRound, ((unit_by_cost ? effs[i] : ents[i]) + T - 1) / T));
                    top.push_back({pr_unit_makespan({ents[i]}, {effs[i]}, {rws[i]}, {}, T, 1 << 14, unit_by_cost, uc), i});
                    (void)k;
                }
                std::sort(top.begin(), top.end(), std::greater<>());
                for (size_t q = 0; q < std::min<size_t>(8, top.size()); q++) {
                    const size_t i = top[q].second;
                    std::fprintf(stderr, "[gx_pr]   block %zu: entries %lld eff %lld rows %lld -> longest unit %.1f us\n", i,
                                 (long long)ents[i], (long long)effs[i], (long long)rws[i], top[q].first);
                }
            }
        }
        GX_HIP_TRY(hipStreamSynchronize(s));
        clk.mark("unit size");
        std::vector<SortedUnit> units;
        int64_t slab = 0;
        int32_t parts = 0;
        for (size_t i = 0; i < sortb.size(); i++) {
            const RowBlock &b = sortb[i];
            const int64_t E = b.nz_end - b.nz_begin;
            const int64_t rounds = (E + kRound - 1) / kRound;
            const int64_t Ek = unit_by_cost ? eff_entries((int64_t)i) : E;
            const int32_t k = (int32_t)std::max<int64_t>(1, std::min<int64_t>(rounds, (Ek + T - 1) / T));
            const int64_t rows_b = b.row_end - b.row_begin;
            for (int32_t j = 0; j < k; j++) {
                SortedUnit u;
                u.lo = b.nz_begin + 256 * (int64_t)h_nsplit[i] + (int64_t)kRound * j;
                u.hi = b.nz_end;
                u.step = (int64_t)kRound * k;
                u.slab = k > 1 ? slab : 0;
                u.nbeg = h_nbeg[i];
                u.nsg = (int32_t)(((int64_t)h_ncode[i] + kNSg - 1) / kNSg);
                u.pbeg = h_pbeg[i];
                u.psg = (int32_t)(((int64_t)h_pcount[i] + kPSg - 1) / kPSg);
                u.pad = 0;
                u.seg = b.seg;
                u.z0 = b.nz_begin;
                u.z1 = b.nz_end;
                u.r0 = b.row_begin;
                u.r1 = b.row_end;
                u.blk = (int32_t)(longb.size() + i);
                u.part = k > 1 ? parts : -1;
                u.unit = j;
                u.nunits = k;
                units.push_back(u);
            }
            if (env_int("GX_PR_VERBOSE", 0, 0, 3) == 3)
                std::fprintf(stderr, "[gx_pr blk] %zu E %lld En %lld codes %u eff %lld k %d rows %lld\n", i, (long long)E,
                             (long long)(std::min<int64_t>(E, 256 * (int64_t)h_nsplit[i]) - std::min<int64_t>(E, 256 * (int64_t)h_psplit[i])), h_ncode[i],
                             (long long)eff_entries((int64_t)i), k, (long long)rows_b);
            if (k > 1) {
                if (p->comb_kernel)
                    for (int64_t s0 = 0; s0 < rows_b; s0 += kCombBS)
                        stripes.push_back({slab, b.row_begin, (int32_t)rows_b, (int32_t)s0,
                                           (int32_t)std::min<int64_t>(rows_b, s0 + kCombBS), k, -1});
                multi[longb.size() + i] = 1;
                slab += (int64_t)k * rows_b;
                parts++;
            }
        }
        const int64_t rowc = env_int("GX_PR_ROW_COST", 4, 0, 1024);
        auto cost = [&](const SortedUnit &u) {
            const RowBlock &b = sortb[u.blk - longb.size()];
            const int64_t E = b.nz_end - b.nz_begin, R = b.row_end - b.row_begin;
            (void)E;
            return (eff_entries(u.blk - (int32_t)longb.size()) + u.nunits - 1) / u.nunits + rowc * R;
        };
        auto iso_unit = [&](const SortedUnit &u) { return iso_block(sortb[u.blk - longb.size()]); };
        std::stable_sort(units.begin(), units.end(), [&](const SortedUnit &x, const SortedUnit &y) {
            const bool ix = iso_unit(x), iy = iso_unit(y);
            if (ix != iy) return iy;
            return cost(x) > cost(y);
        });
        for (const SortedUnit &u : units)
            if (iso_unit(u)) {
                p->iso_units++;
                p->iso_rows += (uint64_t)(u.r1 - u.r0);
            }
        if (p->nlong_pad + (uint32_t)units.size() == p->iso_units) {
            p->iso_units = 0;
            p->iso_rows = 0;
        }
        p->nunits = (uint32_t)units.size();
        if (env_int("GX_PR_VERBOSE", 0, 0, 3))
            std::fprintf(stderr, "[gx_pr] plan: rows %lld nnz %llu unit_nnz %lld block_nnz %d "
                         "long_nnz %d: %zu sorted blocks, %u LONG blocks (%u rows), %u units, %d multi-unit blocks, "
                         "slab %lld doubles; narrow %llu entries in %llu codes\n",
                         (long long)rows, (unsigned long long)nnz, (long long)T,
                         p->sorted_nnz, p->long_nnz, sortb.size(), p->nlong_blocks, p->nlong, p->nunits, parts,
                         (long long)slab, (unsigned long long)p->nnarrow, (unsigned long long)p->ncodes);
        if (env_int("GX_PR_VERBOSE", 0, 0, 3) && pairs_on) {
            size_t nq = 0;
            uint64_t qsum = 0;
            for (uint32_t q : h_psplit) {
                nq += q > 0;
                qsum += q;
            }
            std::fprintf(stderr, "[gx_pr] pairs: %llu entries and %llu filler halves in %llu slots (padding included); "
                         "%zu of %zu blocks with a pair prefix, mean Q %.1f supergroups\n",
                         (unsigned long long)p->npair, (unsigned long long)p->npfill, (unsigned long long)p->npslots, nq,
                         h_psplit.size(), nq ? (double)qsum / (double)nq : 0.0);
        }
        GX_TRY(p->units.alloc(units.size()));
        GX_HIP_TRY(hipMemcpy(p->units.p, units.data(), units.size() * sizeof(SortedUnit), hipMemcpyHostToDevice));
        GX_TRY(p->uslab.alloc(std::max<int64_t>(slab, 1)));
        GX_TRY(p->uticket.alloc(std::max<int32_t>(parts, 1)));
        GX_HIP_TRY(hipMemset(p->uticket.p, 0, p->uticket.n * 4));
    }
    p->unit_nnz = T;
    p->queue_on = env_int("GX_PR_QUEUE", -1, -1, 1);
    GX_TRY(p->queue.alloc(2));
    GX_HIP_TRY(hipMemset(p->queue.p, 0, 2 * sizeof(uint32_t)));
    clk.mark("units");
    {
        std::vector<int32_t> slot(all.size(), -1);
        uint32_t nd = 0;
        auto dangling_in = [&](int64_t r0, int64_t r1) {
            if (p->d_range)
                return p->nd > 0 && r0 < p->d0 + (int64_t)p->nd && r1 > p->d0;
            for (int64_t r2 = r0; r2 < r1; r2++)
                if (h_outdeg[r2] == 0) return true;
            return false;
        };
        for (size_t i = longb.size(); i < all.size(); i++) {
            if (p->comb_kernel && multi[i]) continue;
            if (p->iso_units && iso_block(all[i])) continue;
            if (dangling_in(all[i].row_begin, all[i].row_end)) slot[i] = (int32_t)nd++;
        }
        for (CombStripe &c : stripes)
            if (dangling_in((int64_t)c.r0 + c.s0, (int64_t)c.r0 + c.s1)) c.dslot = (int32_t)nd++;
        for (size_t i = longb.size(); i < all.size() && p->iso_units; i++)
            if (iso_block(all[i])) {
                slot[i] = (int32_t)nd++;
                p->iso_dblocks++;
            }
        p->fused_dangling = p->nd > 0 && nd > 0 && !long_dangling;
        p->ndblocks = nd;
        if (env_int("GX_PR_VERBOSE", 0, 0, 3))
            std::fprintf(stderr, "[gx_pr] closed-form isolated rows: %u of %u units, %llu rows, %u of %u dangling slots\n",
                         p->iso_units, p->nunits, (unsigned long long)p->iso_rows, p->iso_dblocks, nd);
        if (p->fused_dangling) {
            GX_TRY(p->dslot.alloc(std::max<size_t>(all.size(), 1)));
            GX_TRY(p->fdpart.alloc(nd));
            GX_TRY(p->fdticket.alloc(1));
            if (!all.empty()) GX_HIP_TRY(hipMemcpy(p->dslot.p, slot.data(), all.size() * 4, hipMemcpyHostToDevice));
            GX_HIP_TRY(hipMemset(p->fdticket.p, 0, 4));
        }
    }
    p->ncstripes = (uint32_t)stripes.size();
    if (!stripes.empty()) {
        GX_TRY(p->cstripes.alloc(stripes.size()));
        GX_HIP_TRY(hipMemcpy(p->cstripes.p, stripes.data(), stripes.size() * sizeof(CombStripe), hipMemcpyHostToDevice));
    }
    clk.mark("dangling slots");
    return GX_SUCCESS;
}

int pr_step_sorted(PrPart *p, const double *x_full, double *x_local, double *rank_out, hipStream_t s) {
    const double dn = (double)p->n_global;
    SortedArgs a;
    a.blocks = p->blocks.p;
    a.ci = p->ci;
    a.sci = p->sci.p;
    a.spk = p->spk.p;
    a.gbase = p->gbase.p;
    a.outdeg = p->outdeg;
    a.x_in = x_full;
    a.x_out = x_local;
    a.rank_out = rank_out;
    a.chunk = (int64_t)p->chunk;
    a.nranks = p->nranks;
    a.zero_slot = p->nd == 0 ? 1 : 0;
    a.zero_col = (int32_t)p->chunk - 2;
    a.teleport0 = (1.0 - p->damping) / dn;
    a.damping_over_n = p->damping / dn;
    a.damping = p->damping;
    a.long_first = p->long_first.p;
    a.long_nseg = p->long_nseg.p;
    a.long_part = p->long_part.p;
    a.long_ticket = p->long_ticket.p;
    a.nlong = p->nlong_blocks;
    a.nlong_pad = p->nlong_pad;
    a.dslot = p->fused_dangling ? p->dslot.p : nullptr;
    a.dpart = p->fdpart.p;
    a.dticket = p->fdticket.p;
    a.ndblocks = p->ndblocks;
    a.units = p->units.p;
    a.nunits = p->nunits;
    a.uslab = p->uslab.p;
    a.uticket = p->uticket.p;
    a.comb = p->ncstripes > 0 ? 1 : 0;
    a.cstripes = p->cstripes.p;
    a.xd = p->xd.p;
    a.live = (int64_t)p->live;
    a.utimes = nullptr;
    a.npk = p->npk.p;
    a.nbase = p->nbase.p;
    a.null_sg = p->null_sg;
    a.nt_col = p->nt_col;
    a.ppk = p->ppk.p;
    a.pbase = p->pbase.p;
    a.pnull_sg = p->pnull_sg;
    if (p->npair && (reinterpret_cast<uintptr_t>(x_full) & 15))
        return fail(GX_INVALID_VALUE, "pr_step_sorted: pair slots need x 16-byte aligned");
    a.queue = p->queue.p;
    a.iso_rows = 0.0;
    if (!rank_out && p->fused_dangling && p->iso_units) {
        a.nunits -= p->iso_units;
        a.ndblocks -= p->iso_dblocks;
        a.iso_rows = (double)p->iso_rows;
        if (a.ndblocks == 0) a.zero_slot = 1;
    }
    const char *times_path = std::getenv("GX_PR_UNIT_TIMES");
    const uint32_t nw = p->nlong_pad + a.nunits;
    if (times_path && nw) {
        if (!p->utimes.p) GX_TRY(p->utimes.alloc(4 * (size_t)(p->nlong_pad + p->nunits)));
        a.utimes = p->utimes.p;
    }
    if (nw) {
        KTimer kt(p->ctx, "pr_pull", s);
        const size_t lds = (size_t)(1 << kRowBits) * sizeof(double);
        const bool use_queue = p->queue_on == 1 || (p->queue_on == -1 && p->nlong_pad + p->nunits >=
                                                                              2u * (unsigned)std::max(1, p->ctx->num_cus));
        const unsigned nq = std::min<unsigned>(nw, (unsigned)std::max(1, p->ctx->num_cus));
        const PullKernel k = use_queue ? pull_kernel<true>(a.utimes != nullptr, p->cache_policy)
                                       : pull_kernel<false>(a.utimes != nullptr, p->cache_policy);
        hipLaunchKernelGGL(k, dim3(use_queue ? nq : nw), dim3(kBS), lds, s, a);
        if (p->ncstripes) hipLaunchKernelGGL(k_pr_combine, dim3(p->ncstripes), dim3(kCombBS), 0, s, a);
        if (a.utimes && ++p->utimes_launch == env_int("GX_PR_UNIT_TIMES_LAUNCH", 5, 1, 1 << 30)) {
            std::vector<uint64_t> t(4 * (size_t)nw);
            std::vector<SortedUnit> us(p->nunits);
            std::vector<RowBlock> bs(p->nblocks);
            GX_HIP_TRY(hipStreamSynchronize(s));
            GX_HIP_TRY(hipMemcpy(t.data(), p->utimes.p, t.size() * 8, hipMemcpyDeviceToHost));
            if (p->nunits) GX_HIP_TRY(hipMemcpy(us.data(), p->units.p, us.size() * sizeof(SortedUnit), hipMemcpyDeviceToHost));
            if (p->nblocks) GX_HIP_TRY(hipMemcpy(bs.data(), p->blocks.p, bs.size() * sizeof(RowBlock), hipMemcpyDeviceToHost));
            static std::atomic<int> ndump{0};
            char path[512];
            std::snprintf(path, sizeof path, times_path, ndump.fetch_add(1));
            if (FILE *f = std::fopen(path, "w")) {
                std::fprintf(f, "wg kind blk unit nunits entries rows t0 tgather t1 xcc\n");
                for (size_t w = 0; w < nw; w++) {
                    if (w >= p->nlong_blocks && w < p->nlong_pad) continue;
                    const bool lng = w < p->nlong_blocks;
                    long long ents = 0, nrows = 0;
                    int blk = -1, unit = 0, nunits = 1;
                    if (lng) {
                        ents = bs[w].nz_end - bs[w].nz_begin;
                        nrows = 1;
                        blk = (int)w;
                    } else {
                        const SortedUnit &u = us[w - p->nlong_pad];
                        for (int64_t k0 = u.lo; k0 < u.hi; k0 += u.step) ents += std::min<int64_t>(u.step / u.nunits, u.hi - k0);
                        for (int64_t r = u.unit; r * 16 < u.nsg; r += u.nunits)
                            ents += std::min<int64_t>(16, u.nsg - r * 16) * kNSg;
                        for (int64_t r = u.unit; r * 16 < u.psg; r += u.nunits)
                            ents += std::min<int64_t>(16, u.psg - r * 16) * kPSg * 2;
                        blk = u.blk;
                        unit = u.unit;
                        nunits = u.nunits;
                        nrows = bs[u.blk].row_end - bs[u.blk].row_begin;
                    }
                    std::fprintf(f, "%zu %s %d %d %d %lld %lld %llu %llu %llu %llu\n", w,
                                 lng ? "long" : "unit", blk, unit, nunits, ents, nrows,
                                 (unsigned long long)t[4 * w], (unsigned long long)t[4 * w + 1],
                                 (unsigned long long)t[4 * w + 2], (unsigned long long)t[4 * w + 3]);
                }
                std::fclose(f);
            }
        }
    } else if (a.zero_slot) {
        GX_HIP_TRY(hipMemsetAsync(x_local + p->chunk - 1, 0, sizeof(double), s));
    }
    GX_TRY(check_launch("k_pr_pull_units"));
    return p->fused_dangling ? GX_SUCCESS : pr_dangling(p, x_local, s);
}

}

GX_MODULE_WARMER(pr_sorted)
```

Measured before the change: 1084 billion edges/s.

## Add run-group encoding for repeated column pairs in sorted PageRank pull

Adds a new 'run' region ahead of the pair region in each sorted block. Entries that share a column pair are grouped into 64-wide padded groups that hold one pair index and 16-bit row codes. The kernel loads each x pair once per group and broadcasts it across lanes with readlane, instead of gathering x for every entry. This aims to cut redundant gather traffic on columns that appear many times. In exchange it adds padding codes, planning kernels (cost, fill, emit), and a new cost term in unit balancing.

```diff
diff --git a/ldbc_graphalytics_platforms_graphblas_amd/csrc/gx_pr.h b/ldbc_graphalytics_platforms_graphblas_amd/csrc/gx_pr.h
--- a/ldbc_graphalytics_platforms_graphblas_amd/csrc/gx_pr.h
+++ b/ldbc_graphalytics_platforms_graphblas_amd/csrc/gx_pr.h
@@ -60,7 +60,8 @@
     int32_t r0, r1;
     int64_t pbeg;
     int32_t psg;
-    int32_t pad;
+    int32_t rsg;
+    int64_t rbeg;
 };
 
 struct CombStripe {
@@ -122,6 +123,12 @@
     uint64_t npfill = 0;
     uint64_t npslots = 0;
     uint32_t pnull_sg = 0;
+    DBuf<uint16_t> rpk;
+    DBuf<uint32_t> rpair;
+    uint64_t nrun = 0;
+    uint64_t nrpad = 0;
+    uint64_t nrcodes = 0;
+    uint32_t rnull_sg = 0;
     int sorted_nnz = 65536;
     int sorted_rows = 4096;
     int64_t unit_nnz = 0;
diff --git a/ldbc_graphalytics_platforms_graphblas_amd/csrc/gx_pr_runs.h b/ldbc_graphalytics_platforms_graphblas_amd/csrc/gx_pr_runs.h
--- /dev/null
+++ b/ldbc_graphalytics_platforms_graphblas_amd/csrc/gx_pr_runs.h
@@ -0,0 +1,36 @@
+#pragma once
+
+#include <cstdint>
+
+#if defined(__HIPCC__)
+#define GX_RUN_HD __host__ __device__ __forceinline__
+#else
+#define GX_RUN_HD inline
+#endif
+
+namespace gx {
+
+constexpr int kRunGroup = 64;
+constexpr int kRunSg = 512;
+constexpr int kRunSgGroups = kRunSg / kRunGroup;
+
+GX_RUN_HD uint32_t run_pad(uint64_t len) { return (uint32_t)((0 - len) & (uint64_t)(kRunGroup - 1)); }
+
+GX_RUN_HD uint64_t run_code_pos(uint64_t e, uint64_t pad_before) { return e + pad_before; }
+
+struct RunCursor {
+    uint64_t pad;
+    GX_RUN_HD uint64_t place(uint64_t e) const { return run_code_pos(e, pad); }
+    GX_RUN_HD void end_run(uint64_t len) { pad += run_pad(len); }
+};
+
+GX_RUN_HD uint64_t run_group_of(uint64_t pos) { return pos / kRunGroup; }
+
+GX_RUN_HD uint64_t run_slot(uint64_t pos) {
+    return (pos & ~(uint64_t)(kRunSg - 1)) + (pos & (uint64_t)(kRunGroup - 1)) * kRunSgGroups +
+           ((pos / kRunGroup) & (uint64_t)(kRunSgGroups - 1));
+}
+
+GX_RUN_HD uint64_t run_region_codes(uint64_t end_pos) { return (end_pos + kRunGroup - 1) / kRunGroup * kRunGroup; }
+
+}
diff --git a/ldbc_graphalytics_platforms_graphblas_amd/csrc/gx_pr_sorted.hip b/ldbc_graphalytics_platforms_graphblas_amd/csrc/gx_pr_sorted.hip
--- a/ldbc_graphalytics_platforms_graphblas_amd/csrc/gx_pr_sorted.hip
+++ b/ldbc_graphalytics_platforms_graphblas_amd/csrc/gx_pr_sorted.hip
@@ -9,6 +9,7 @@
 
 #include "gx_pr.h"
 #include "gx_pr_bank.h"
+#include "gx_pr_runs.h"
 
 namespace gx {
 namespace {
@@ -20,6 +21,8 @@
 constexpr int kRound = kBS * kU;
 constexpr int kNSg = 512;
 constexpr int kPSg = 256;
+constexpr int kRunFillCost = 32;
+constexpr int kRunCost = 2;
 constexpr int kJunkRow = (1 << kRowBits) - kWave;
 constexpr int kMaxBlockRows = kJunkRow;
 static_assert(kMaxBlockRows == kPlanBlockRows, "gx_pr.h block rows");
@@ -61,6 +64,9 @@
     const uint32_t *ppk;
     const uint32_t *pbase;
     uint32_t pnull_sg;
+    const uint16_t *rpk;
+    const uint32_t *rpair;
+    uint32_t rnull_sg;
     double *xd;
     int64_t live;
     uint32_t *queue;
@@ -490,6 +496,85 @@
     }
 }
 
+template <int CP>
+__device__ __forceinline__ void gather_runs(const SortedArgs &a, const SortedUnit &u, double *acc) {
+    constexpr int W = kBS / kWave;
+    const int32_t nrounds = (u.rsg + W - 1) / W;
+    if (u.unit >= nrounds) return;
+    const int32_t nr = (nrounds - u.unit + u.nunits - 1) / u.nunits;
+    const int tid = threadIdx.x;
+    const int lane = tid & (kWave - 1);
+    const int wave = tid >> 6;
+    const uint32_t sg0 = (uint32_t)(u.rbeg / kRunSg);
+    const char *xb = reinterpret_cast<const char *>(a.x_in);
+    typedef uint32_t u32x4 __attribute__((ext_vector_type(4)));
+    typedef double d2 __attribute__((ext_vector_type(2)));
+    struct Rd {
+        u32x4 q;
+        uint32_t pair;
+    };
+    struct Gt {
+        d2 g;
+        uint32_t c[4];
+    };
+    auto load = [&](Rd &d, int32_t i) {
+        const int32_t sg = (u.unit + i * u.nunits) * W + wave;
+        const uint32_t g = sg < u.rsg ? sg0 + (uint32_t)sg : a.rnull_sg;
+        const u32x4 *qa = reinterpret_cast<const u32x4 *>(a.rpk + (size_t)g * kRunSg) + lane;
+        d.q = (CP & 1) ? __builtin_nontemporal_load(qa) : *qa;
+        d.pair = a.rpair[(size_t)g * kRunSgGroups + (lane & (kRunSgGroups - 1))];
+    };
+    auto issue = [&](const Rd &d, Gt &t) {
+        const uint32_t w[4] = {d.q.x, d.q.y, d.q.z, d.q.w};
+#pragma unroll
+        for (int k = 0; k < 4; k++) {
+            t.c[k] = w[k];
+            asm volatile("" : "+v"(t.c[k]));
+        }
+        t.g = *reinterpret_cast<const d2 *>(xb + (d.pair << 4));
+    };
+    auto add = [&](const Gt &t) {
+        const int xl = __double2loint(t.g.x), xh = __double2hiint(t.g.x);
+        const int yl = __double2loint(t.g.y), yh = __double2hiint(t.g.y);
+#pragma unroll
+        for (int k = 0; k < kRunSgGroups; k++) {
+            const double xk = __hiloint2double(__builtin_amdgcn_readlane(xh, k), __builtin_amdgcn_readlane(xl, k));
+            const double yk = __hiloint2double(__builtin_amdgcn_readlane(yh, k), __builtin_amdgcn_readlane(yl, k));
+            const uint32_t c = (k & 1) ? (t.c[k >> 1] >> 16) : (t.c[k >> 1] & 0xffffu);
+            atomicAdd(&acc[c & ((1u << kRowBits) - 1)], (c & (1u << kRowBits)) ? yk : xk);
+        }
+    };
+    Rd dA, dB;
+    Gt tA, tB;
+    load(dA, 0);
+    load(dB, 1);
+    issue(dA, tA);
+    __builtin_amdgcn_sched_barrier(0);
+    load(dA, 2);
+    int32_t k = 1;
+    for (; k + 1 < nr; k += 2) {
+        __builtin_amdgcn_sched_barrier(0);
+        issue(dB, tB);
+        __builtin_amdgcn_sched_barrier(0);
+        load(dB, k + 2);
+        __builtin_amdgcn_sched_barrier(0);
+        add(tA);
+        __builtin_amdgcn_sched_barrier(0);
+        issue(dA, tA);
+        __builtin_amdgcn_sched_barrier(0);
+        load(dA, k + 3);
+        __builtin_amdgcn_sched_barrier(0);
+        add(tB);
+    }
+    if (k < nr) {
+        issue(dB, tB);
+        add(tA);
+        add(tB);
+    } else {
+        add(tA);
+    }
+}
+
 template <bool TIMES, int CP>
 __device__ __forceinline__ void pull_item(const SortedArgs &a, const uint32_t w, double *acc, double *wred, int &last,
                                           const double teleport) {
@@ -517,6 +602,7 @@
     if (!empty) {
         for (int i = tid; i < nrows; i += kBS) acc[i] = 0.0;
         __syncthreads();
+        gather_runs<CP>(a, u, acc);
         gather_pairs<CP>(a, u, acc);
         gather_narrow<CP>(a, u, acc);
         gather_units<CP>(a, b, u.lo, u.hi, acc, u.step);
@@ -838,13 +924,15 @@
 }
 
 constexpr int kBankTile = 2048, kBankBS = 256, kBankPer = kBankTile / kBankBS;
-__global__ __launch_bounds__(kBankBS) void k_bank_order(const RowBlock *__restrict__ blocks, const uint32_t *__restrict__ qsplit,
+__global__ __launch_bounds__(kBankBS) void k_bank_order(const RowBlock *__restrict__ blocks, const uint32_t *__restrict__ rsplit,
+                                                        const uint32_t *__restrict__ qsplit,
                                                         const uint32_t *__restrict__ nsplit, uint32_t *spk, int32_t *sci) {
     __shared__ uint32_t cnt2[kBankTile / 2][kBankClasses / 2];
     __shared__ int32_t wred[2][kBankBS / kWave];
     const RowBlock b = blocks[blockIdx.y];
     const int64_t z0 = b.nz_begin, N = b.nz_end - z0;
     const int64_t Nq = min(N, (int64_t)qsplit[blockIdx.y] << 8), Np = min(N, (int64_t)nsplit[blockIdx.y] << 8);
+    const int64_t Nr = min(N, (int64_t)rsplit[blockIdx.y] << 8);
     const int64_t ntiles = (Np + kBankTile - 1) / kBankTile;
     const int tid = threadIdx.x, lane = tid & (kWave - 1), wave = tid / kWave;
     for (int64_t g = blockIdx.x; g < ntiles; g += gridDim.x) {
@@ -872,7 +960,7 @@
 #pragma unroll
         for (int j = 0; j < kBankPer; j++) {
             const int32_t i = i0 + j;
-            head[j] = i == 0 || i >= nin || t0 + i == Nq || key[j] != (j ? key[j - 1] : prevkey);
+            head[j] = i == 0 || i >= nin || t0 + i == Nq || t0 + i == Nr || key[j] != (j ? key[j - 1] : prevkey);
             if (head[j]) last = i;
             s0[j] = last;
         }
@@ -924,8 +1012,8 @@
                 cnt[2 * k + 1] = w >> 16;
             }
             const uint32_t k = bank_deal_pos(cnt, p[j] & (uint32_t)(kBankClasses - 1), rank[j]);
-            const bool pairs = t0 + s0[j] < Nq;
-            const int64_t dst = z0 + t0 + s0[j] + (pairs ? bank_pair_pos(k, n) : k);
+            const bool pairs = t0 + s0[j] < Nq, runs = t0 + s0[j] < Nr;
+            const int64_t dst = z0 + t0 + s0[j] + (pairs && !runs ? bank_pair_pos(k, n) : k);
             spk[dst] = p[j];
             if (pairs) sci[dst] = c[j];
         }
@@ -1088,6 +1176,18 @@
     bool in[4], start[4], lead[4], half[4];
 };
 
+__device__ __forceinline__ int64_t pair_run_start(const int32_t *__restrict__ sci, int64_t z0, int64_t f) {
+    const uint32_t pf = (uint32_t)sci[z0 + f] >> 1;
+    if (f == 0 || ((uint32_t)sci[z0 + f - 1] >> 1) != pf) return f;
+    int64_t lo = 0, hi = f;
+    while (lo < hi) {
+        const int64_t mid = (lo + hi) >> 1;
+        if (((uint32_t)sci[z0 + mid] >> 1) >= pf) hi = mid;
+        else lo = mid + 1;
+    }
+    return lo;
+}
+
 __device__ __forceinline__ void pair_lane(const int32_t *__restrict__ sci, int64_t z0, int64_t N, int64_t Nq, int64_t g,
                                           int lane, PairLane &o) {
     const int64_t i0 = (g << 8) + 4 * lane;
@@ -1095,17 +1195,7 @@
 #pragma unroll
     for (int j = 0; j < 6; j++) c[j] = (uint32_t)sci[z0 + min(max(i0 + j - 1, (int64_t)0), N - 1)];
     const int64_t f = g << 8;
-    const uint32_t pf = (uint32_t)sci[z0 + f] >> 1;
-    int64_t gs = f;
-    if (f > 0 && ((uint32_t)sci[z0 + f - 1] >> 1) == pf) {
-        int64_t lo = 0, hi = f;
-        while (lo < hi) {
-            const int64_t mid = (lo + hi) >> 1;
-            if (((uint32_t)sci[z0 + mid] >> 1) >= pf) hi = mid;
-            else lo = mid + 1;
-        }
-        gs = lo;
-    }
+    const int64_t gs = pair_run_start(sci, z0, f);
     int32_t ls = -1;
 #pragma unroll
     for (int j = 0; j < 4; j++) {
@@ -1139,9 +1229,11 @@
 }
 
 __global__ __launch_bounds__(256) void k_pair_cost(const RowBlock *__restrict__ blocks, const int32_t *__restrict__ sci,
-                                                   uint32_t *__restrict__ slots, uint32_t *__restrict__ fill) {
+                                                   const uint32_t *__restrict__ rsplit, uint32_t *__restrict__ slots,
+                                                   uint32_t *__restrict__ fill) {
     const RowBlock b = blocks[blockIdx.y];
-    const int64_t z0 = b.nz_begin, N = b.nz_end - z0, ng = (N + 255) >> 8;
+    const int64_t R = rsplit[blockIdx.y];
+    const int64_t z0 = b.nz_begin + (R << 8), N = b.nz_end - z0, ng = (N + 255) >> 8;
     const int lane = threadIdx.x & (kWave - 1);
     const int64_t waves = (int64_t)gridDim.x * blockDim.x / kWave;
     for (int64_t g = ((int64_t)blockIdx.x * blockDim.x + threadIdx.x) / kWave; g < ng; g += waves) {
@@ -1156,8 +1248,8 @@
         ns = wave_total(ns);
         nf = wave_total(nf);
         if (lane == 0) {
-            slots[b.seg + g] = ns;
-            fill[b.seg + g] = nf;
+            slots[b.seg + R + g] = ns;
+            fill[b.seg + R + g] = nf;
         }
     }
 }
@@ -1172,12 +1264,14 @@
 }
 
 __global__ __launch_bounds__(256) void k_pair_emit(const RowBlock *__restrict__ blocks, const int32_t *__restrict__ sci,
-                                                   const uint32_t *__restrict__ spk, const uint32_t *__restrict__ qsplit,
+                                                   const uint32_t *__restrict__ spk, const uint32_t *__restrict__ rsplit,
+                                                   const uint32_t *__restrict__ qsplit,
                                                    const uint32_t *__restrict__ pcount, const uint32_t *__restrict__ poff,
                                                    const int64_t *__restrict__ pbeg, uint32_t *__restrict__ ppk,
                                                    uint32_t *__restrict__ pbase, unsigned long long *__restrict__ nfill) {
     const RowBlock b = blocks[blockIdx.y];
-    const int64_t z0 = b.nz_begin, N = b.nz_end - z0, Q = qsplit[blockIdx.y];
+    const int64_t R = rsplit[blockIdx.y];
+    const int64_t z0 = b.nz_begin + (R << 8), N = b.nz_end - z0, Q = (int64_t)qsplit[blockIdx.y] - R;
     const int64_t Nq = min(N, Q << 8);
     const int64_t pb = pbeg[blockIdx.y], C = pcount[blockIdx.y];
     const int lane = threadIdx.x & (kWave - 1);
@@ -1193,7 +1287,7 @@
             n += (pl.lead[j] ? 1u : 0u) + (pl.start[j] ? pl.sf[j] : 0u);
             nf += (pl.half[j] ? 1u : 0u) + (pl.start[j] ? 2 * pl.sf[j] : 0u);
         }
-        int64_t pos = pb + poff[b.seg + g] + (wave_scan_incl(n) - n);
+        int64_t pos = pb + poff[b.seg + R + g] + (wave_scan_incl(n) - n);
         nf = wave_total(nf);
         if (lane == 0 && nf) atomicAdd(nfill, (unsigned long long)nf);
         auto put = [&](uint32_t step, uint32_t ha, uint32_t hb, uint32_t pair_after) {
@@ -1220,6 +1314,103 @@
             const uint32_t hb = pl.half[j] ? (uint32_t)(kJunkRow + (pos & (kWave - 1)))
                                            : ((pl.next[j] & 1u) << kRowBits) | (spk[z0 + e + 1] & kRowMask);
             put(step, ha, hb, pl.pair[j]);
+        }
+    }
+}
+
+
+struct RunLane {
+    uint32_t pair[4], col[4], len[4];
+    bool in[4];
+};
+
+__device__ __forceinline__ void run_lane(const int32_t *__restrict__ sci, int64_t z0, int64_t N, int64_t Nr, int64_t g,
+                                         int lane, RunLane &o) {
+    const int64_t i0 = (g << 8) + 4 * lane;
+    uint32_t c[6];
+#pragma unroll
+    for (int j = 0; j < 6; j++) c[j] = (uint32_t)sci[z0 + min(max(i0 + j - 1, (int64_t)0), N - 1)];
+    const int64_t f = g << 8;
+    const int64_t gs = pair_run_start(sci, z0, f);
+    bool start[4];
+    int32_t ls = -1;
+#pragma unroll
+    for (int j = 0; j < 4; j++) {
+        const int64_t i = i0 + j;
+        o.in[j] = i < Nr;
+        o.col[j] = c[j + 1];
+        o.pair[j] = c[j + 1] >> 1;
+        start[j] = o.in[j] && (i == 0 || (c[j] >> 1) != o.pair[j]);
+        if (start[j]) ls = 4 * lane + j;
+    }
+    int32_t m = ls;
+#pragma unroll
+    for (int d = 1; d < kWave; d <<= 1) {
+        const int32_t v = __shfl_up(m, d, kWave);
+        if (lane >= d) m = max(m, v);
+    }
+    int32_t before = __shfl_up(m, 1, kWave);
+    if (lane == 0) before = -1;
+    int64_t rs = before >= 0 ? f + before : gs;
+#pragma unroll
+    for (int j = 0; j < 4; j++) {
+        const int64_t i = i0 + j;
+        if (start[j]) rs = i;
+        const bool end = o.in[j] && (i + 1 >= Nr || (c[j + 2] >> 1) != o.pair[j]);
+        o.len[j] = end ? (uint32_t)(i - rs + 1) : 0u;
+    }
+}
+
+__global__ __launch_bounds__(256) void k_run_cost(const RowBlock *__restrict__ blocks, const int32_t *__restrict__ sci,
+                                                  uint32_t *__restrict__ fill) {
+    const RowBlock b = blocks[blockIdx.y];
+    const int64_t z0 = b.nz_begin, N = b.nz_end - z0, ng = (N + 255) >> 8;
+    const int lane = threadIdx.x & (kWave - 1);
+    const int64_t waves = (int64_t)gridDim.x * blockDim.x / kWave;
+    for (int64_t g = ((int64_t)blockIdx.x * blockDim.x + threadIdx.x) / kWave; g < ng; g += waves) {
+        RunLane rl;
+        run_lane(sci, z0, N, N, g, lane, rl);
+        RunCursor cur{0};
+#pragma unroll
+        for (int j = 0; j < 4; j++) cur.end_run(rl.len[j]);
+        const uint32_t nf = wave_total((uint32_t)cur.pad);
+        if (lane == 0) fill[b.seg + g] = nf;
+    }
+}
+
+__global__ void k_run_fill(uint16_t *__restrict__ rpk, uint64_t ncodes, uint32_t *__restrict__ rpair, uint32_t zero_pair) {
+    for (uint64_t p = (uint64_t)blockIdx.x * blockDim.x + threadIdx.x; p < ncodes; p += (uint64_t)gridDim.x * blockDim.x) {
+        rpk[p] = (uint16_t)(kJunkRow + ((p / kRunSgGroups) & (kWave - 1)));
+        if ((p & (kRunGroup - 1)) == 0) rpair[p / kRunGroup] = zero_pair;
+    }
+}
+
+__global__ __launch_bounds__(256) void k_run_emit(const RowBlock *__restrict__ blocks, const int32_t *__restrict__ sci,
+                                                  const uint32_t *__restrict__ spk, const uint32_t *__restrict__ rsplit,
+                                                  const uint32_t *__restrict__ roff, const int64_t *__restrict__ rbeg,
+                                                  uint16_t *__restrict__ rpk, uint32_t *__restrict__ rpair) {
+    const RowBlock b = blocks[blockIdx.y];
+    const int64_t z0 = b.nz_begin, N = b.nz_end - z0, R = rsplit[blockIdx.y];
+    const int64_t Nr = min(N, R << 8);
+    const int64_t rb = rbeg[blockIdx.y];
+    const int lane = threadIdx.x & (kWave - 1);
+    const int64_t waves = (int64_t)gridDim.x * blockDim.x / kWave;
+    for (int64_t g = ((int64_t)blockIdx.x * blockDim.x + threadIdx.x) / kWave; g < R; g += waves) {
+        RunLane rl;
+        run_lane(sci, z0, N, Nr, g, lane, rl);
+        RunCursor lanepad{0};
+#pragma unroll
+        for (int j = 0; j < 4; j++) lanepad.end_run(rl.len[j]);
+        const uint32_t n = (uint32_t)lanepad.pad;
+        RunCursor cur{(uint64_t)roff[b.seg + g] - (uint64_t)(g << 8) + (wave_scan_incl(n) - n)};
+#pragma unroll
+        for (int j = 0; j < 4; j++) {
+            const int64_t e = (g << 8) + 4 * lane + j;
+            if (!rl.in[j]) continue;
+            const uint64_t pos = (uint64_t)rb + cur.place((uint64_t)e);
+            rpk[run_slot(pos)] = (uint16_t)(((rl.col[j] & 1u) << kRowBits) | (spk[z0 + e] & ((1u << kRowBits) - 1)));
+            if ((pos & (kRunGroup - 1)) == 0) rpair[run_group_of(pos)] = rl.pair[j];
+            cur.end_run(rl.len[j]);
         }
     }
 }
@@ -1388,8 +1579,13 @@
     p->ncodes = 0;
     p->nnarrow = 0;
     p->npair = p->npfill = p->npslots = 0;
+    p->nrun = p->nrpad = p->nrcodes = 0;
+    std::vector<uint32_t> h_rsplit(sortb.size(), 0), h_rcode(sortb.size(), 0);
+    std::vector<int64_t> h_rbeg(sortb.size(), 0);
     const bool pairs_on = env_int("GX_PR_PAIRS", huge && !piece ? 1 : 0, 0, 1) == 1;
     if (pairs_on && (p->chunk & 1)) return fail(GX_INVALID_VALUE, "pr_plan_sorted: pair slots need an even chunk");
+    const bool runs_on = env_int("GX_PR_RUNS", huge && !piece ? 1 : 0, 0, 1) == 1;
+    if (runs_on && (p->chunk & 1)) return fail(GX_INVALID_VALUE, "pr_plan_sorted: run groups need an even chunk");
     DBuf<int32_t> d_seg_row;
     DBuf<SegDesc> d_segd;
     DBuf<int64_t> srow;
@@ -1400,6 +1596,8 @@
     DBuf<uint32_t> d_pslots, d_pfill, d_poff, d_psplit, d_pcount;
     DBuf<int64_t> d_pbeg;
     DBuf<unsigned long long> d_npfill;
+    DBuf<uint32_t> d_rfill, d_roff, d_rsplit, d_rcode;
+    DBuf<int64_t> d_rbeg;
     if (nnz > 0) {
         std::vector<std::pair<int32_t, int32_t>> order_;
         for (size_t i = 0; i < sortb.size(); i++) order_.push_back({sortb[i].row_begin, (int32_t)i});
@@ -1511,16 +1709,33 @@
             GX_TRY(d_pcount.alloc(nsb));
             GX_TRY(d_pbeg.alloc(nsb));
             GX_TRY(d_npfill.alloc(1));
-            GX_HIP_TRY(hipMemsetAsync(d_psplit.p, 0, nsb * 4, s));
             GX_HIP_TRY(hipMemsetAsync(d_npfill.p, 0, sizeof(unsigned long long), s));
+            GX_TRY(d_rsplit.alloc(nsb));
+            GX_HIP_TRY(hipMemsetAsync(d_rsplit.p, 0, nsb * 4, s));
+            if (runs_on) {
+                GX_TRY(d_rfill.alloc(std::max<int64_t>(ngroups, 1)));
+                GX_TRY(d_roff.alloc(std::max<int64_t>(ngroups, 1)));
+                GX_TRY(d_rcode.alloc(nsb));
+                GX_TRY(d_rbeg.alloc(nsb));
+                hipLaunchKernelGGL(k_run_cost, dim3(64, nsb), dim3(256), 0, s, d_sort, p->sci.p, d_rfill.p);
+                GX_TRY(check_launch("k_run_cost"));
+                hipLaunchKernelGGL(k_narrow_split, dim3(nsb), dim3(1024), 0, s, d_sort, d_rfill.p, (const uint32_t *)nullptr,
+                                   env_int("GX_PR_RUN_FILL_COST", kRunFillCost, 0, 1 << 20), (const uint32_t *)nullptr, 1,
+                                   (int64_t)env_int("GX_PR_RUN_MIN", 65536, 0, 1 << 30), d_rsplit.p, d_rcode.p, d_roff.p);
+                GX_TRY(check_launch("k_narrow_split (runs)"));
+                GX_HIP_TRY(hipMemcpyAsync(h_rsplit.data(), d_rsplit.p, nsb * 4, hipMemcpyDeviceToHost, s));
+                GX_HIP_TRY(hipMemcpyAsync(h_rcode.data(), d_rcode.p, nsb * 4, hipMemcpyDeviceToHost, s));
+            }
+            GX_HIP_TRY(hipMemcpyAsync(d_psplit.p, d_rsplit.p, nsb * 4, hipMemcpyDeviceToDevice, s));
             if (pairs_on) {
                 GX_TRY(d_pslots.alloc(std::max<int64_t>(ngroups, 1)));
                 GX_TRY(d_pfill.alloc(std::max<int64_t>(ngroups, 1)));
                 GX_TRY(d_poff.alloc(std::max<int64_t>(ngroups, 1)));
-                hipLaunchKernelGGL(k_pair_cost, dim3(64, nsb), dim3(256), 0, s, d_sort, p->sci.p, d_pslots.p, d_pfill.p);
+                hipLaunchKernelGGL(k_pair_cost, dim3(64, nsb), dim3(256), 0, s, d_sort, p->sci.p, d_rsplit.p, d_pslots.p,
+                                   d_pfill.p);
                 GX_TRY(check_launch("k_pair_cost"));
                 hipLaunchKernelGGL(k_narrow_split, dim3(nsb), dim3(1024), 0, s, d_sort, d_pfill.p, d_pslots.p,
-                                   env_int("GX_PR_PAIR_FILL_COST", 48, 0, 1 << 20), (const uint32_t *)nullptr, 1,
+                                   env_int("GX_PR_PAIR_FILL_COST", 48, 0, 1 << 20), d_rsplit.p, 1,
                                    (int64_t)env_int("GX_PR_PAIR_MIN", 0, 0, 1 << 30), d_psplit.p, d_pcount.p, d_poff.p);
                 GX_TRY(check_launch("k_narrow_split (pairs)"));
                 GX_HIP_TRY(hipMemcpyAsync(h_psplit.data(), d_psplit.p, nsb * 4, hipMemcpyDeviceToHost, s));
@@ -1535,23 +1750,46 @@
             GX_HIP_TRY(hipMemcpyAsync(h_nsplit.data(), d_nsplit.p, nsb * 4, hipMemcpyDeviceToHost, s));
             GX_HIP_TRY(hipMemcpyAsync(h_ncode.data(), d_ncode.p, nsb * 4, hipMemcpyDeviceToHost, s));
             GX_HIP_TRY(hipStreamSynchronize(s));
-            uint64_t run = 0, prun = 0;
+            if (!pairs_on) h_psplit = h_rsplit;
+            uint64_t run = 0, prun = 0, rrun = 0;
             for (size_t i = 0; i < sortb.size(); i++) {
                 const int64_t E = sortb[i].nz_end - sortb[i].nz_begin;
+                const int64_t Er = std::min<int64_t>((int64_t)h_rsplit[i] * 256, E);
                 const int64_t Ep = std::min<int64_t>((int64_t)h_psplit[i] * 256, E);
+                h_rcode[i] = (uint32_t)run_region_codes(h_rcode[i]);
+                h_rbeg[i] = (int64_t)rrun;
+                rrun += ((uint64_t)h_rcode[i] + kRunSg - 1) / kRunSg * kRunSg;
+                p->nrun += (uint64_t)Er;
+                p->nrpad += (uint64_t)h_rcode[i] - (uint64_t)Er;
                 h_nbeg[i] = (int64_t)run;
                 run += ((uint64_t)h_ncode[i] + kNSg - 1) / kNSg * kNSg;
                 p->nnarrow += (uint64_t)(std::min<int64_t>((int64_t)h_nsplit[i] * 256, E) - Ep);
                 h_pbeg[i] = (int64_t)prun;
                 prun += ((uint64_t)h_pcount[i] + kPSg - 1) / kPSg * kPSg;
-                p->npair += (uint64_t)Ep;
+                p->npair += (uint64_t)(Ep - Er);
             }
             if (env_int("GX_PR_BANK_ORDER", huge && !piece ? 1 : 0, 0, 1) == 1) {
                 clk.mark("prefix splits");
-                hipLaunchKernelGGL(k_bank_order, dim3(64, nsb), dim3(kBankBS), 0, s, d_sort, d_psplit.p, d_nsplit.p, p->spk.p,
-                                   p->sci.p);
+                hipLaunchKernelGGL(k_bank_order, dim3(64, nsb), dim3(kBankBS), 0, s, d_sort, d_rsplit.p, d_psplit.p, d_nsplit.p,
+                                   p->spk.p, p->sci.p);
                 GX_TRY(check_launch("k_bank_order"));
                 clk.mark("bank order");
+            }
+            if (runs_on) {
+                p->rnull_sg = (uint32_t)(rrun / kRunSg);
+                p->nrcodes = rrun + kRunSg;
+                GX_TRY(p->rpk.alloc(p->nrcodes, 16));
+                GX_TRY(p->rpair.alloc(p->nrcodes / kRunGroup));
+                hipLaunchKernelGGL(k_run_fill, dim3(grid_for(p->nrcodes, 256, 16384)), dim3(256), 0, s, p->rpk.p, p->nrcodes,
+                                   p->rpair.p, (uint32_t)((p->chunk - 2) >> 1));
+                GX_TRY(check_launch("k_run_fill"));
+                if (p->nrun) {
+                    GX_HIP_TRY(hipMemcpyAsync(d_rbeg.p, h_rbeg.data(), nsb * 8, hipMemcpyHostToDevice, s));
+                    hipLaunchKernelGGL(k_run_emit, dim3(64, nsb), dim3(256), 0, s, d_sort, p->sci.p, p->spk.p, d_rsplit.p,
+                                       d_roff.p, d_rbeg.p, p->rpk.p, p->rpair.p);
+                    GX_TRY(check_launch("k_run_emit"));
+                }
+                clk.mark("run codes");
             }
             p->pnull_sg = (uint32_t)(prun / kPSg);
             p->npslots = prun + kPSg;
@@ -1562,7 +1800,7 @@
             GX_TRY(check_launch("k_pair_fill"));
             if (p->npair) {
                 GX_HIP_TRY(hipMemcpyAsync(d_pbeg.p, h_pbeg.data(), nsb * 8, hipMemcpyHostToDevice, s));
-                hipLaunchKernelGGL(k_pair_emit, dim3(64, nsb), dim3(256), 0, s, d_sort, p->sci.p, p->spk.p, d_psplit.p,
+                hipLaunchKernelGGL(k_pair_emit, dim3(64, nsb), dim3(256), 0, s, d_sort, p->sci.p, p->spk.p, d_rsplit.p, d_psplit.p,
                                    d_pcount.p, d_poff.p, d_pbeg.p, p->ppk.p, p->pbase.p, d_npfill.p);
                 GX_TRY(check_launch("k_pair_emit"));
                 unsigned long long nf = 0;
@@ -1599,14 +1837,18 @@
     const bool cost_codes = env_int("GX_PR_COST_CODES", piece ? 1 : 0, 0, 1) == 1;
     const int64_t fill_cost4 = env_int("GX_PR_FILL_COST", 4, 0, 64);
     const int64_t pair_cost4 = env_int("GX_PR_PAIR_COST", 4, 1, 64);
+    const int64_t run_cost4 = env_int("GX_PR_RUN_COST", kRunCost, 1, 64);
     auto eff_entries = [&](int64_t i) -> int64_t {
         const int64_t E = sortb[i].nz_end - sortb[i].nz_begin;
-        const int64_t Ep = std::min<int64_t>(E, 256 * (int64_t)h_psplit[i]);
+        const int64_t Er = std::min<int64_t>(E, 256 * (int64_t)h_rsplit[i]);
+        const int64_t Erp = std::min<int64_t>(E, 256 * (int64_t)h_psplit[i]);
+        const int64_t Ep = Erp - Er;
         const int64_t Enp = std::min<int64_t>(E, 256 * (int64_t)h_nsplit[i]);
-        const int64_t En = Enp - Ep;
+        const int64_t En = Enp - Erp;
         const int64_t fill = cost_codes ? std::max<int64_t>(0, (int64_t)h_ncode[i] - En) : 0;
         const int64_t pent = cost_codes ? std::max<int64_t>(Ep, 2 * (int64_t)h_pcount[i]) : Ep;
-        return pent * pair_cost4 / 4 + En + fill * fill_cost4 / 4 + (E - Enp) * wide_cost4 / 4;
+        return (int64_t)h_rcode[i] * run_cost4 / 4 + pent * pair_cost4 / 4 + En + fill * fill_cost4 / 4 +
+               (E - Enp) * wide_cost4 / 4;
     };
     const bool unit_by_cost = env_int("GX_PR_UNIT_BY_COST", huge ? 1 : 0, 0, 1) == 1;
     p->comb_kernel = env_int("GX_PR_COMBINE", piece ? 1 : 0, 0, 1) == 1;
@@ -1711,7 +1953,8 @@
                 u.nsg = (int32_t)(((int64_t)h_ncode[i] + kNSg - 1) / kNSg);
                 u.pbeg = h_pbeg[i];
                 u.psg = (int32_t)(((int64_t)h_pcount[i] + kPSg - 1) / kPSg);
-                u.pad = 0;
+                u.rbeg = h_rbeg[i];
+                u.rsg = (int32_t)(((int64_t)h_rcode[i] + kRunSg - 1) / kRunSg);
                 u.seg = b.seg;
                 u.z0 = b.nz_begin;
                 u.z1 = b.nz_end;
@@ -1770,7 +2013,8 @@
         if (env_int("GX_PR_VERBOSE", 0, 0, 3) && pairs_on) {
             size_t nq = 0;
             uint64_t qsum = 0;
-            for (uint32_t q : h_psplit) {
+            for (size_t i = 0; i < h_psplit.size(); i++) {
+                const uint32_t q = h_psplit[i] - h_rsplit[i];
                 nq += q > 0;
                 qsum += q;
             }
@@ -1778,6 +2022,18 @@
                          "%zu of %zu blocks with a pair prefix, mean Q %.1f supergroups\n",
                          (unsigned long long)p->npair, (unsigned long long)p->npfill, (unsigned long long)p->npslots, nq,
                          h_psplit.size(), nq ? (double)qsum / (double)nq : 0.0);
+        }
+        if (env_int("GX_PR_VERBOSE", 0, 0, 3)) {
+            size_t nq = 0;
+            uint64_t rsum = 0;
+            for (uint32_t q : h_rsplit) {
+                nq += q > 0;
+                rsum += q;
+            }
+            std::fprintf(stderr, "[gx_pr] runs: %llu entries and %llu padding codes in %llu codes (supergroup padding "
+                         "included); %zu of %zu blocks with a run prefix, mean R %.1f supergroups\n",
+                         (unsigned long long)p->nrun, (unsigned long long)p->nrpad, (unsigned long long)p->nrcodes, nq,
+                         h_rsplit.size(), nq ? (double)rsum / (double)nq : 0.0);
         }
         GX_TRY(p->units.alloc(units.size()));
         GX_HIP_TRY(hipMemcpy(p->units.p, units.data(), units.size() * sizeof(SortedUnit), hipMemcpyHostToDevice));
@@ -1879,8 +2135,11 @@
     a.ppk = p->ppk.p;
     a.pbase = p->pbase.p;
     a.pnull_sg = p->pnull_sg;
-    if (p->npair && (reinterpret_cast<uintptr_t>(x_full) & 15))
-        return fail(GX_INVALID_VALUE, "pr_step_sorted: pair slots need x 16-byte aligned");
+    a.rpk = p->rpk.p;
+    a.rpair = p->rpair.p;
+    a.rnull_sg = p->rnull_sg;
+    if ((p->npair || p->nrun) && (reinterpret_cast<uintptr_t>(x_full) & 15))
+        return fail(GX_INVALID_VALUE, "pr_step_sorted: pair slots and run groups need x 16-byte aligned");
     a.queue = p->queue.p;
     a.iso_rows = 0.0;
     if (!rank_out && p->fused_dangling && p->iso_units) {
@@ -1932,6 +2191,8 @@
                         for (int64_t k0 = u.lo; k0 < u.hi; k0 += u.step) ents += std::min<int64_t>(u.step / u.nunits, u.hi - k0);
                         for (int64_t r = u.unit; r * 16 < u.nsg; r += u.nunits)
                             ents += std::min<int64_t>(16, u.nsg - r * 16) * kNSg;
+                        for (int64_t r = u.unit; r * 16 < u.rsg; r += u.nunits)
+                            ents += std::min<int64_t>(16, u.rsg - r * 16) * kRunSg;
                         for (int64_t r = u.unit; r * 16 < u.psg; r += u.nunits)
                             ents += std::min<int64_t>(16, u.psg - r * 16) * kPSg * 2;
                         blk = u.blk;
```

Result: faster. 1156 billion edges/s (median of 6 runs) (+6.6%).
